# uthree/ALiVE-VC

Hardware: AMD Instinct MI355X
Metric: VC frames/sec + RTF @24kHz, 1M-vec library; 1/2/4/8 MI355X (higher is better)
Workload: dtype decoder fp16 GEMMs / fp32 acc; encoders 22-bit fp16 split; kNN exact fp32 top-k via fp6 MFMA candidates (certified); f32 MFMA small convs; f64 phase scan

## Files before the change

### alive-vc_amd/csrc/gemm_planes.hip

```cpp
#include "conv_epilogue.h"
#include "planes_layout.h"

namespace {

constexpr int GM = 128, GN = 128, GK = 32;
constexpr int PLANE_BYTES = GM * GK * 2;

typedef const __attribute__((address_space(1))) void* gptr_t;
typedef __attribute__((address_space(3))) void* lptr_t;

template <int N>
__device__ __forceinline__ void wait_vmcnt() {
    __builtin_amdgcn_s_waitcnt((N & 15) | (7 << 4) | (15 << 8) | ((N >> 4) << 14));
}
__device__ __forceinline__ void wait_lgkmcnt0() { __builtin_amdgcn_s_waitcnt(15 | (7 << 4) | (0 << 8) | (3 << 14)); }

struct GemmWalk {
    int64_t a_ks, b_blk, b_tap;
    int ncb;
    int rg, n_ct;
};
__device__ __forceinline__ void tile_of(int v, int n_mt, const GemmWalk& g, int& mt, int& ct) {
    const int gs = g.rg * g.n_ct;
    const int grp = v / gs, rem = v - grp * gs;
    const int left = n_mt - grp * g.rg;
    const int rows = left < g.rg ? left : g.rg;
    ct = rem / rows;
    mt = grp * g.rg + (rem - ct * rows);
}
struct StepWalk {
    int64_t a = 0, b = 0;
    int blk = 0;
    __device__ __forceinline__ void reset() { a = 0; b = 0; blk = 0; }
    __device__ __forceinline__ void advance(const GemmWalk& g) {
        a += g.a_ks;
        b += g.b_blk;
        if (++blk == g.ncb) { blk = 0; b += g.b_tap - (int64_t)g.ncb * g.b_blk; }
    }
};

template <int NP>
__device__ __forceinline__ unsigned pack_plane2(float a, float b, bool count = true) { return NP == 1 ? pack_f16x2(a, b, count) : pack_bf16x2(a, b); }
template <int NP, bool F16S>
__device__ __forceinline__ unsigned split_step(float& a, float& b, bool count = true) {
    if constexpr (F16S) {
        typedef _Float16 f16x2_t __attribute__((ext_vector_type(2)));
        const unsigned h = pack_f16x2(a, b, count);
        const f16x2_t hv = __builtin_bit_cast(f16x2_t, h);
        a -= (float)hv[0];
        b -= (float)hv[1];
        return h;
    } else {
        const unsigned h = pack_plane2<NP>(a, b, count);
        a -= __uint_as_float(h << 16);
        b -= __uint_as_float(h & 0xffff0000u);
        return h;
    }
}

template <int NP, int ACT, bool F16S = false>
__device__ __forceinline__ void gemm_epilogue(const AliveGemm& p, f32x16 (&acc)[2][2], int m0, int64_t c0, int wr, int wc, int lr,
                                              int lh, int64_t cols, int64_t cols_pad, int co_pad32, unsigned char* stage = nullptr,
                                              unsigned char* stage_small = nullptr) {
    if constexpr (ACT == 3) {
        float bv[2] = {-INFINITY, -INFINITY};
        int bi[2] = {0x7fffffff, 0x7fffffff};
        auto take = [](float v, int vi, float b, int i) { return argmax_takes(v, vi, b, i); };
#pragma unroll
        for (int ti = 0; ti < 2; ++ti) {
            const int rbase = m0 + wr * 64 + ti * 32 + 4 * lh;
#pragma unroll
            for (int r = 0; r < 16; ++r) {
                const int row = rbase + (r & 3) + 8 * (r >> 2);
                const float b = p.bias != nullptr ? p.bias[row < p.Co ? row : p.Co - 1] : 0.0f;
                const float osc = F16S ? p.wscale[0] * p.in_unscale : 1.0f;
#pragma unroll
                for (int tj = 0; tj < 2; ++tj) {
                    const float x = F16S ? fmaf(acc[ti][tj][r], osc, b) : acc[ti][tj][r] + b;
                    if (row < p.Co && take(x, row, bv[tj], bi[tj])) { bv[tj] = x; bi[tj] = row; }
                }
            }
        }
        const int blk = (m0 + wr * 64) >> 6;
#pragma unroll
        for (int tj = 0; tj < 2; ++tj) {
            const float ov = __shfl_xor(bv[tj], 32);
            const int oi = __shfl_xor(bi[tj], 32);
            if (take(ov, oi, bv[tj], bi[tj])) { bv[tj] = ov; bi[tj] = oi; }
            const int64_t col = c0 + wc * 64 + tj * 32 + lr;
            if (lh == 0 && col < cols && m0 + wr * 64 < p.Co) {
                p.arg_val[(size_t)blk * cols + col] = bv[tj];
                p.arg_idx[(size_t)blk * cols + col] = bi[tj];
            }
        }
        return;
    }
    if constexpr (ACT == 4) {
        unsigned char* st = stage_small != nullptr ? stage_small : stage;
        unsigned short* Po = (unsigned short*)p.Pout;
        const int bins = p.Co >> 1;
        const int bin0 = (m0 + wr * 64) >> 1;
        const int lane = lr + 32 * lh;
#pragma unroll
        for (int tj = 0; tj < 2; ++tj) {
            float q[2][4][2];
#pragma unroll
            for (int ti = 0; ti < 2; ++ti)
#pragma unroll
                for (int g = 0; g < 4; ++g)
#pragma unroll
                    for (int e = 0; e < 2; ++e) {
                        const int bin = bin0 + 16 * ti + 4 * g + 2 * lh + e;
                        const float m = hypotf(acc[ti][tj][4 * g + 2 * e], acc[ti][tj][4 * g + 2 * e + 1]);
                        q[ti][g][e] = bin < bins ? m : 0.0f;
                    }
#pragma unroll
            for (int pl = 0; pl < NP; ++pl) {
#pragma unroll
                for (int ti = 0; ti < 2; ++ti)
#pragma unroll
                    for (int g = 0; g < 4; ++g) {
                        const unsigned h = pack_plane2<NP>(q[ti][g][0], q[ti][g][1]);
                        *(unsigned*)(st + lr * 64 + (((2 * ti + (g >> 1)) ^ ((lr >> 2) & 3)) << 4) + 8 * (g & 1) + 4 * lh) = h;
                        q[ti][g][0] -= __uint_as_float(h << 16);
                        q[ti][g][1] -= __uint_as_float(h & 0xffff0000u);
                    }
#pragma unroll
                for (int it = 0; it < 2; ++it) {
                    const int idx = it * 64 + lane, cl = idx >> 2, chunk = idx & 3;
                    const u32x4 v = *(const u32x4*)(st + cl * 64 + ((chunk ^ ((cl >> 2) & 3)) << 4));
                    const int64_t col = c0 + wc * 64 + tj * 32 + cl;
                    const int b = bin0 + chunk * 8;
                    if (col < cols_pad && b < co_pad32) *(u32x4*)(Po + planes_at(pl, col, b, cols_pad, co_pad32)) = col < cols ? v : u32x4{0u, 0u, 0u, 0u};
                }
            }
        }
        return;
    }
    const bool second = p.y_split > 0 && m0 >= p.y_split;
    float* const Yout = second ? p.Y2 : p.Y;
    const int row_off = second ? p.y_split : 0;
    const int co_out = p.y_split > 0 ? (second ? p.Co - p.y_split : p.y_split) : p.Co;
    unsigned obase[2];
    bool cok[2];
#pragma unroll
    for (int tj = 0; tj < 2; ++tj) {
        const int64_t col = c0 + wc * 64 + tj * 32 + lr;
        cok[tj] = col < cols;
        const int64_t n = cok[tj] ? col / p.T : 0;
        obase[tj] = (unsigned)(n * co_out * p.T + (cok[tj] ? col - n * p.T : 0)) - (unsigned)(row_off * p.T);
    }
    const bool full_rows = m0 + GM <= p.Co;
    const float oscale = F16S ? p.wscale[0] * p.in_unscale : 1.0f;
    const float pscale = F16S ? p.pout_scale : 1.0f;
    const float* __restrict__ bias = p.bias;
    const float* __restrict__ post_add = p.post_add;
    const float* __restrict__ ch_scale = p.ch_scale;
#pragma unroll
    for (int ti = 0; ti < 2; ++ti) {
        const int rbase = m0 + wr * 64 + ti * 32 + 4 * lh;
        float bia[4][4], pad[4][4], scl[4][4];
#pragma unroll
        for (int g = 0; g < 4; ++g)
#pragma unroll
            for (int e = 0; e < 4; ++e) {
                int row = rbase + 8 * g + e;
                row = row < p.Co ? row : p.Co - 1;
                bia[g][e] = bias != nullptr ? bias[row] : 0.0f;
                pad[g][e] = post_add != nullptr ? post_add[row] : 0.0f;
                scl[g][e] = ch_scale != nullptr ? ch_scale[row] : 1.0f;
            }
        float res[2][16];
        if (p.residual != nullptr) {
#pragma unroll
            for (int tj = 0; tj < 2; ++tj)
#pragma unroll
                for (int r = 0; r < 16; ++r) {
                    int row = rbase + (r & 3) + 8 * (r >> 2);
                    row = row < p.Co ? row : p.Co - 1;
                    res[tj][r] = p.residual[obase[tj] + (unsigned)(row * p.T)];
                }
        }
#pragma unroll
        for (int tj = 0; tj < 2; ++tj) {
            float vv[16];
#pragma unroll
            for (int r = 0; r < 16; ++r) {
                float x = F16S ? fmaf(acc[ti][tj][r], oscale, bia[r >> 2][r & 3]) : acc[ti][tj][r] + bia[r >> 2][r & 3];
                if (ACT == 1) x = gelu_fast(x);
                else if (ACT == 2) x = expf(x);
                x = (x + pad[r >> 2][r & 3]) * scl[r >> 2][r & 3];
                if (p.residual != nullptr) x += res[tj][r];
                vv[r] = x;
            }
            if (Yout != nullptr && cok[tj]) {
                if (full_rows) {
#pragma unroll
                    for (int r = 0; r < 16; ++r)
                        Yout[obase[tj] + (unsigned)((rbase + (r & 3) + 8 * (r >> 2)) * p.T)] = vv[r];
                } else {
#pragma unroll
                    for (int r = 0; r < 16; ++r) {
                        const int row = rbase + (r & 3) + 8 * (r >> 2);
                        if (row < p.Co) Yout[obase[tj] + (unsigned)(row * p.T)] = vv[r];
                    }
                }
            }
            if (p.Pout != nullptr && stage != nullptr) {
                const int cl = tj * 32 + lr;
#pragma unroll
                for (int g = 0; g < 4; ++g) {
                    const int rowl = ti * 32 + 8 * g + 4 * lh;
                    float q[4];
#pragma unroll
                    for (int e = 0; e < 4; ++e) q[e] = (full_rows || rbase + 8 * g + e < p.Co) ? vv[4 * g + e] * pscale : 0.0f;
#pragma unroll
                    for (int pl = 0; pl < NP; ++pl) {
                        const unsigned h01 = split_step<NP, F16S>(q[0], q[1], cok[tj]), h23 = split_step<NP, F16S>(q[2], q[3], cok[tj]);
                        *(uint2*)(stage + pl * 8192 + cl * 128 + ((((rowl >> 3)) ^ (cl & 7)) << 4) + 8 * lh) = make_uint2(h01, h23);
                    }
                }
            } else if (p.Pout != nullptr && stage_small != nullptr) {
                unsigned short* Po = (unsigned short*)p.Pout;
                float q[4][4];
#pragma unroll
                for (int g = 0; g < 4; ++g)
#pragma unroll
                    for (int e = 0; e < 4; ++e) q[g][e] = (full_rows || rbase + 8 * g + e < p.Co) ? vv[4 * g + e] * pscale : 0.0f;
                const int lane = lr + 32 * lh;
#pragma unroll
                for (int pl = 0; pl < NP; ++pl) {
#pragma unroll
                    for (int g = 0; g < 4; ++g) {
                        const unsigned h01 = split_step<NP, F16S>(q[g][0], q[g][1], cok[tj]), h23 = split_step<NP, F16S>(q[g][2], q[g][3], cok[tj]);
                        *(uint2*)(stage_small + lr * 64 + ((g ^ ((lr >> 2) & 3)) << 4) + 8 * lh) = make_uint2(h01, h23);
                    }
#pragma unroll
                    for (int it = 0; it < 2; ++it) {
                        const int idx = it * 64 + lane, cl = idx >> 2, chunk = idx & 3;
                        const u32x4 v = *(const u32x4*)(stage_small + cl * 64 + ((chunk ^ ((cl >> 2) & 3)) << 4));
                        const int64_t col = c0 + wc * 64 + tj * 32 + cl;
                        const int row0 = m0 + wr * 64 + ti * 32 + chunk * 8;
                        if (col < cols && row0 < co_pad32) *(u32x4*)(Po + planes_at(pl, col, row0, cols_pad, co_pad32)) = v;
                    }
                }
            }
        }
    }
    if (p.Pout != nullptr && stage != nullptr) {
        unsigned short* Po = (unsigned short*)p.Pout;
        const int lane = lr + 32 * lh;
#pragma unroll
        for (int it = 0; it < 8; ++it) {
            const int cl = (it & 3) * 16 + (lane >> 2), chunk = (it >> 2) * 4 + (lane & 3);
            const int64_t col = c0 + wc * 64 + cl;
            const int row0 = m0 + wr * 64 + chunk * 8;
            if (col >= cols || row0 >= co_pad32) continue;
#pragma unroll
            for (int pl = 0; pl < NP; ++pl) {
                const u32x4 v = *(const u32x4*)(stage + pl * 8192 + cl * 128 + ((chunk ^ (cl & 7)) << 4));
                *(u32x4*)(Po + planes_at(pl, col, row0, cols_pad, co_pad32)) = v;
            }
        }
    }
}

template <int NP, int NS, int MINB, int ACT, bool KB2 = false, bool F16S = false>
__global__ __launch_bounds__(256, MINB) void gemm_planes_kernel(AliveGemm p, int n_mt, int ntiles, int64_t cols,
                                                             int64_t cols_pad, int co_pad, int co_pad32, int kpad,
                                                             GemmWalk gw, long long* stamps) {
#ifdef ALIVE_STAMPS
    const long long ts0 = wall_clock64();
#endif
    extern __shared__ __attribute__((aligned(16))) unsigned char smem[];
    constexpr int SLOT = 2 * NP * PLANE_BYTES;
    constexpr int NI = 4 * NP;
    constexpr int NPROD = KB2 ? 2 : NP * (NP + 1) / 2;
    static_assert(!KB2 || NP == 2, "the 64-deep one-plane form lives in the two-plane kernel's slots");
    static_assert(!F16S || (NP == 2 && !KB2), "fp16 split planes: two planes, 32-deep steps");

    const int tid = threadIdx.x, lane = tid & 63;
    const int w = __builtin_amdgcn_readfirstlane(tid >> 6);
    const int wr = w >> 1, wc = w & 1;
    const int lr = lane & 31, lh = lane >> 5;

    int v;
    {
        const int L = blockIdx.x, xcd = L & 7, j = L >> 3, q = ntiles >> 3, r = ntiles & 7;
        v = (xcd < r ? xcd * (q + 1) : r * (q + 1) + (xcd - r) * q) + j;
    }
    int mt, ct;
    tile_of(v, n_mt, gw, mt, ct);
    const int m0 = mt * GM;
    const int64_t c0 = (int64_t)ct * GN;
    const int nsteps = kpad / (KB2 ? 2 * GK : GK);

    const int prow = lane >> 2;
    const int pchunk = (lane & 3) ^ ((prow >> 2) & 3);
    const unsigned short* src[NI];
    int ldst[NI];
#pragma unroll
    for (int i = 0; i < NI; ++i) {
        const int q = w + 4 * i;
        const int op = q / (8 * NP), pl = (q % (8 * NP)) / 8, g = q % 8;
        const int spl = KB2 ? 0 : pl;
        const int r = g * 16 + prow;
        if (op == 0) {
            int row = m0 + r;
            row = row < co_pad ? row : co_pad - 1;
            src[i] = (const unsigned short*)p.W + planes_at(spl, row, 0, co_pad, kpad) + pchunk * 8;
        } else if (p.b_row == 0) {
            int64_t col = c0 + r;
            col = col < cols_pad ? col : cols_pad - 1;
            src[i] = (const unsigned short*)p.P + planes_at(spl, col, 0, cols_pad, kpad) + pchunk * 8;
        } else {
            int64_t col = c0 + r;
            col = col < cols ? col : cols - 1;
            const int64_t nn = col / p.T;
            src[i] = (const unsigned short*)p.P + (size_t)spl * p.b_plane + (size_t)nn * p.b_win + (size_t)(col - nn * p.T) * p.b_row + pchunk * 8;
        }
        ldst[i] = (op * NP + pl) * PLANE_BYTES + g * 1024;
    }
    StepWalk walk, walk1;
    if constexpr (KB2) walk1.advance(gw);
    auto issue = [&](int step, int i) {
        const StepWalk& wk = (KB2 && ((i >> 1) & 1)) ? walk1 : walk;
        __builtin_amdgcn_global_load_lds((gptr_t)(src[i] + (i < 2 * NP ? wk.a : wk.b)), (lptr_t)(smem + (step % NS) * SLOT + ldst[i]), 16, 0, 0);
    };
    auto next_step = [&]() {
        walk.advance(gw);
        if constexpr (KB2) { walk.advance(gw); walk1.advance(gw); walk1.advance(gw); }
    };

    f32x16 acc[2][2];
#pragma unroll
    for (int i = 0; i < 2; ++i)
#pragma unroll
        for (int r = 0; r < 16; ++r) { acc[i][0][r] = 0.0f; acc[i][1][r] = 0.0f; }

#pragma unroll
    for (int s = 0; s < NS; ++s)
        if (s < nsteps) {
#pragma unroll
            for (int i = 0; i < NI; ++i) issue(s, i);
            next_step();
        }

    const int sw = (lr >> 2) & 3;
    const int a_off = (wr * 64 + lr) * 64 + ((lh ^ sw) << 4);
    const int b_off = NP * PLANE_BYTES + (wc * 64 + lr) * 64 + ((lh ^ sw) << 4);

    bf16x8 fa[2][2][NP], fb[2][2][NP];
    auto load_frags = [&](int step, int ks, bf16x8 (&a)[2][NP], bf16x8 (&b)[2][NP]) {
        const unsigned char* S = smem + (step % NS) * SLOT;
#pragma unroll
        for (int t = 0; t < 2; ++t)
#pragma unroll
            for (int pl = 0; pl < NP; ++pl) {
                a[t][pl] = *(const bf16x8*)(S + ((a_off + t * 2048) ^ (ks << 5)) + pl * PLANE_BYTES);
                b[t][pl] = *(const bf16x8*)(S + ((b_off + t * 2048) ^ (ks << 5)) + pl * PLANE_BYTES);
            }
    };
    auto mma = [&](bf16x8 (&a)[2][NP], bf16x8 (&b)[2][NP], auto&& hook) {
        int n = 0;
        if constexpr (KB2) {
#pragma unroll
            for (int kb = 0; kb < 2; ++kb) {
#pragma unroll
                for (int ti = 0; ti < 2; ++ti)
#pragma unroll
                    for (int tj = 0; tj < 2; ++tj) acc[ti][tj] = mfma_f16(a[ti][kb], b[tj][kb], acc[ti][tj]);
                hook(n++);
            }
            return;
        }
#pragma unroll
        for (int sum = NP - 1; sum >= 0; --sum)
#pragma unroll
            for (int i = 0; i <= sum; ++i) {
#pragma unroll
                for (int ti = 0; ti < 2; ++ti)
#pragma unroll
                    for (int tj = 0; tj < 2; ++tj)
                        acc[ti][tj] = (NP == 1 || F16S) ? mfma_f16(a[ti][i], b[tj][sum - i], acc[ti][tj])
                                                        : __builtin_amdgcn_mfma_f32_32x32x16_bf16(a[ti][i], b[tj][sum - i], acc[ti][tj], 0, 0, 0);
                hook(n++);
            }
    };

#ifdef ALIVE_STAMPS
    const long long ts1 = wall_clock64();
#endif
    if (nsteps >= NS) wait_vmcnt<(NS - 1) * NI>(); else wait_vmcnt<0>();
    __builtin_amdgcn_s_barrier();
    load_frags(0, 0, fa[0], fb[0]);
#ifdef ALIVE_STAMPS
    const long long ts2 = wall_clock64();
    long long cy_vm = 0, cy_bar = 0;
    const long long cy_l0 = __builtin_readcyclecounter();
#endif

    for (int s = 0; s < nsteps; ++s) {
        mma(fa[0], fb[0], [&](int n) {
            if (n == 0) load_frags(s, 1, fa[1], fb[1]);
        });
        __builtin_amdgcn_sched_barrier(0);
        wait_lgkmcnt0();
#ifdef ALIVE_STAMPS
        const long long cy0 = __builtin_readcyclecounter();
#endif
        if (s + NS - 1 < nsteps) wait_vmcnt<(NS - 2) * NI>(); else wait_vmcnt<0>();
#ifdef ALIVE_STAMPS
        const long long cy1 = __builtin_readcyclecounter();
#endif
        __builtin_amdgcn_s_barrier();
#ifdef ALIVE_STAMPS
        const long long cy2 = __builtin_readcyclecounter();
        cy_vm += cy1 - cy0; cy_bar += cy2 - cy1;
#endif
        if (s + 1 < nsteps) load_frags(s + 1, 0, fa[0], fb[0]);
        __builtin_amdgcn_sched_barrier(0);
        const bool refill = s + NS < nsteps;
        mma(fa[1], fb[1], [&](int n) {
#pragma unroll
            for (int i = 0; i < NI; ++i)
                if (i * NPROD / NI == n && refill) issue(s + NS, i);
        });
        next_step();
        __builtin_amdgcn_sched_barrier(0);
    }
    wait_vmcnt<0>();
#ifdef ALIVE_STAMPS
    const long long ts3 = wall_clock64();
    const long long cy_l1 = __builtin_readcyclecounter();
#endif

    unsigned char* stage = nullptr;
    if constexpr (ACT != 3) {
        if (p.Pout != nullptr) {
            __syncthreads();
            stage = smem + w * (NP * 8192);
        }
    }
    gemm_epilogue<KB2 ? 1 : NP, ACT, F16S>(p, acc, m0, c0, wr, wc, lr, lh, cols, cols_pad, co_pad32, stage);
#ifdef ALIVE_STAMPS
    if (stamps != nullptr && tid == 0) {
        long long* o = stamps + (size_t)blockIdx.x * 8;
        o[0] = ts0; o[1] = ts1; o[2] = ts2; o[3] = ts3; o[4] = wall_clock64();
        o[5] = cy_l1 - cy_l0;
        o[6] = cy_vm; o[7] = cy_bar;
    }
#endif
}

template <int NP, int NS, int ACT>
__global__ __launch_bounds__(512, 1) void gemm_planes_lw_kernel(AliveGemm p, int n_mt, int ntiles, int64_t cols, int64_t cols_pad,
                                                                int co_pad, int co_pad32, int kpad, GemmWalk gw) {
    extern __shared__ __attribute__((aligned(16))) unsigned char smem[];
    constexpr int SLOT = 2 * NP * PLANE_BYTES;
    constexpr int NI = 4 * NP;
    [[maybe_unused]] constexpr int NPROD = NP * (NP + 1) / 2;

    const int tid = threadIdx.x, lane = tid & 63;
    const int w8 = __builtin_amdgcn_readfirstlane(tid >> 6);
    const int nsteps = kpad / GK;

    int v, v_end;
    const int v_stride = gridDim.x >> 3;
    {
        const int xcd = blockIdx.x & 7, j = blockIdx.x >> 3, q = ntiles >> 3, r = ntiles & 7;
        const int beg = xcd < r ? xcd * (q + 1) : r * (q + 1) + (xcd - r) * q;
        v_end = beg + q + (xcd < r ? 1 : 0);
        v = beg + j;
    }
    if (v >= v_end) return;

    if (w8 >= 4) {
        const int w = w8 - 4;
        const int prow = lane >> 2;
        const int pchunk = (lane & 3) ^ ((prow >> 2) & 3);
        int ldst[NI];
        unsigned off[2][NI];
#pragma unroll
        for (int i = 0; i < NI; ++i) {
            const int q = w + 4 * i;
            ldst[i] = ((i >= 2 * NP ? NP : 0) + (q % (8 * NP)) / 8) * PLANE_BYTES + (q % 8) * 1024;
        }
        auto tile_offsets = [&](int tv, unsigned (&o)[NI]) {
            int mt, ct;
            tile_of(tv, n_mt, gw, mt, ct);
            const int64_t c0 = (int64_t)ct * GN;
#pragma unroll
            for (int i = 0; i < NI; ++i) {
                const int q = w + 4 * i;
                const int pl = (q % (8 * NP)) / 8, r = (q % 8) * 16 + prow;
                if (i < 2 * NP) {
                    int row = mt * GM + r;
                    row = row < co_pad ? row : co_pad - 1;
                    o[i] = (unsigned)((planes_at(pl, row, 0, co_pad, kpad) + pchunk * 8) * 2);
                } else if (p.b_row == 0) {
                    int64_t col = c0 + r;
                    col = col < cols_pad ? col : cols_pad - 1;
                    o[i] = (unsigned)((planes_at(pl, col, 0, cols_pad, kpad) + pchunk * 8) * 2);
                } else {
                    int64_t col = c0 + r;
                    col = col < cols ? col : cols - 1;
                    const int64_t nn = col / p.T;
                    o[i] = (unsigned)(((size_t)pl * p.b_plane + (size_t)nn * p.b_win + (size_t)(col - nn * p.T) * p.b_row + pchunk * 8) * 2);
                }
            }
        };
        StepWalk walk;
        auto issue = [&](int which, int slot, int i) {
            const unsigned char* base = i >= 2 * NP ? (const unsigned char*)p.P : (const unsigned char*)p.W;
            __builtin_amdgcn_global_load_lds((gptr_t)(base + off[which][i] + (unsigned)((i >= 2 * NP ? walk.b : walk.a) * 2)),
                                             (lptr_t)(smem + slot * SLOT + ldst[i]), 16, 0, 0);
        };
        int cur = 0, qb = 0;
        tile_offsets(v, off[0]);
#pragma unroll
        for (int s = 0; s < NS; ++s) {
#pragma unroll
            for (int i = 0; i < NI; ++i) issue(0, s, i);
            walk.advance(gw);
        }
        wait_vmcnt<(NS - 1) * NI>();
        __builtin_amdgcn_s_barrier();
        while (true) {
            const int vn = v + v_stride;
            const bool has_next = vn < v_end;
            if (has_next) tile_offsets(vn, off[cur ^ 1]);
            for (int s = 0; s < nsteps; ++s) {
                const int slot = (qb + s) % NS;
                if (s + NS - 1 < nsteps || has_next) wait_vmcnt<(NS - 2) * NI>(); else wait_vmcnt<0>();
                __builtin_amdgcn_s_barrier();
                const int ts = s + NS;
                const bool in_tile = ts < nsteps;
                if (ts == nsteps) walk.reset();
                if (in_tile || has_next) {
#pragma unroll
                    for (int i = 0; i < NI; ++i) issue(in_tile ? cur : (cur ^ 1), slot, i);
                }
                walk.advance(gw);
            }
            if (!has_next) break;
            v = vn;
            cur ^= 1;
            qb = (qb + nsteps) % NS;
        }
        return;
    }

    const int w = w8;
    const int wr = w >> 1, wc = w & 1;
    const int lr = lane & 31, lh = lane >> 5;
    const int sw = (lr >> 2) & 3;
    const int a_off = (wr * 64 + lr) * 64 + ((lh ^ sw) << 4);
    const int b_off = NP * PLANE_BYTES + (wc * 64 + lr) * 64 + ((lh ^ sw) << 4);
    bf16x8 fa[2][2][NP], fb[2][2][NP];
    auto load_frags = [&](int slot, int ks, bf16x8 (&a)[2][NP], bf16x8 (&b)[2][NP]) {
        const unsigned char* S = smem + slot * SLOT;
#pragma unroll
        for (int t = 0; t < 2; ++t)
#pragma unroll
            for (int pl = 0; pl < NP; ++pl) {
                a[t][pl] = *(const bf16x8*)(S + ((a_off + t * 2048) ^ (ks << 5)) + pl * PLANE_BYTES);
                b[t][pl] = *(const bf16x8*)(S + ((b_off + t * 2048) ^ (ks << 5)) + pl * PLANE_BYTES);
            }
    };
    f32x16 acc[2][2];
    auto mma = [&](bf16x8 (&a)[2][NP], bf16x8 (&b)[2][NP], auto&& hook) {
        int n = 0;
#pragma unroll
        for (int sum = NP - 1; sum >= 0; --sum)
#pragma unroll
            for (int i = 0; i <= sum; ++i) {
#pragma unroll
                for (int ti = 0; ti < 2; ++ti)
#pragma unroll
                    for (int tj = 0; tj < 2; ++tj)
                        acc[ti][tj] = NP == 1 ? mfma_f16(a[ti][i], b[tj][sum - i], acc[ti][tj])
                                              : __builtin_amdgcn_mfma_f32_32x32x16_bf16(a[ti][i], b[tj][sum - i], acc[ti][tj], 0, 0, 0);
                hook(n++);
            }
    };

    int qb = 0;
    __builtin_amdgcn_s_barrier();
    while (true) {
        const int vn = v + v_stride;
        const bool has_next = vn < v_end;
#pragma unroll
        for (int i = 0; i < 2; ++i)
#pragma unroll
            for (int r = 0; r < 16; ++r) { acc[i][0][r] = 0.0f; acc[i][1][r] = 0.0f; }
        load_frags(qb, 0, fa[0], fb[0]);
        for (int s = 0; s < nsteps; ++s) {
            const int slot = (qb + s) % NS;
            const int slot1 = slot + 1 == NS ? 0 : slot + 1;
            mma(fa[0], fb[0], [&](int n) {
                if (n == 0) load_frags(slot, 1, fa[1], fb[1]);
            });
            __builtin_amdgcn_sched_barrier(0);
            wait_lgkmcnt0();
            __builtin_amdgcn_s_barrier();
            if (s + 1 < nsteps) load_frags(slot1, 0, fa[0], fb[0]);
            __builtin_amdgcn_sched_barrier(0);
            mma(fa[1], fb[1], [&](int) {});
            __builtin_amdgcn_sched_barrier(0);
        }
        {
            int mt, ct;
            tile_of(v, n_mt, gw, mt, ct);
            gemm_epilogue<NP, ACT>(p, acc, mt * GM, (int64_t)ct * GN, wr, wc, lr, lh, cols, cols_pad, co_pad32, nullptr,
                                   p.Pout != nullptr ? smem + NS * SLOT + w * 2048 : nullptr);
        }
        if (!has_next) break;
        v = vn;
        qb = (qb + nsteps) % NS;
    }
}

template <int NP>
__global__ __launch_bounds__(256) void to_planes_kernel(const float* __restrict__ X, int C, int T, int64_t cols, int64_t cols_pad,
                                                        int c_pad, unsigned short* __restrict__ P) {
    __shared__ float tile[64][65];
    const int lane = threadIdx.x & 63, wv = threadIdx.x >> 6;
    const int64_t col0 = (int64_t)blockIdx.x * 64;
    const int ch0 = blockIdx.y * 64;
    {
        const int64_t col = col0 + lane;
        const bool ok = col < cols;
        const int64_t n = ok ? col / T : 0;
        const int t = ok ? (int)(col - n * T) : 0;
        const float* xc = X + (size_t)n * C * T + t;
        for (int r = wv; r < 64; r += 4) {
            const int c = ch0 + r;
            tile[r][lane] = (ok && c < C) ? xc[(size_t)c * T] : 0.0f;
        }
    }
    __syncthreads();
#pragma unroll
    for (int it = 0; it < 2; ++it) {
        const int item = it * 256 + threadIdx.x;
        const int ck = it * 4 + (item & 3), cl = (item >> 2) & 63;
        const int64_t col = col0 + cl;
        const int c = ch0 + ck * 8;
        if (col >= cols_pad || c >= c_pad) continue;
        float vv[8];
#pragma unroll
        for (int e = 0; e < 8; ++e) vv[e] = tile[ck * 8 + e][cl];
#pragma unroll
        for (int pl = 0; pl < NP; ++pl) {
            u32x4 o;
#pragma unroll
            for (int e = 0; e < 4; ++e) {
                const unsigned h = pack_plane2<NP>(vv[2 * e], vv[2 * e + 1]);
                o[e] = h;
                vv[2 * e] -= __uint_as_float(h << 16);
                vv[2 * e + 1] -= __uint_as_float(h & 0xffff0000u);
            }
            *(u32x4*)(P + planes_at(pl, col, c, cols_pad, c_pad)) = o;
        }
    }
}

long long* g_stamps = nullptr;
inline int64_t pad_cols(int64_t cols) { return (cols + GN - 1) / GN * GN; }
inline int pad32(int c) { return (c + 31) & ~31; }
inline GemmWalk make_walk(const AliveGemm& d) {
    GemmWalk g;
    g.a_ks = (int64_t)((d.Co + 15) & ~15) * GK;
    if (d.b_row == 0) { g.b_blk = pad_cols((int64_t)d.N * d.T) * GK; g.b_tap = 0; g.ncb = pad32(d.Ci) / GK; }
    else if (d.b_cblk == 0) { g.b_blk = 0; g.b_tap = GK; g.ncb = 1; }
    else { g.b_blk = d.b_blk; g.b_tap = GK; g.ncb = d.b_cblk; }
    static const int rg_env = getenv("ALIVE_GEMM_RG") ? atoi(getenv("ALIVE_GEMM_RG")) : 0;
    const int n_mt = cdiv(d.Co, GM);
    const int64_t tile_bytes = (int64_t)GM * pad32(d.Ci) * d.planes * 2;
    int rg = rg_env > 0 ? rg_env : (int)std::max<int64_t>(1, (int64_t)(2.5 * 1048576) / tile_bytes);
    rg = std::min(rg, n_mt);
    const int n_rg = cdiv(n_mt, rg);
    g.rg = cdiv(n_mt, n_rg);
    g.n_ct = cdiv((int64_t)d.N * d.T, GN);
    return g;
}

template <int NP, int NS, int MINB, int ACT, bool KB2 = false, bool F16S = false>
int launch_gemm_act(const AliveGemm& d, hipStream_t s) {
    constexpr int LDS = NS * 2 * NP * PLANE_BYTES;
    {
        static LdsOptIn optin;
        hipError_t e = optin.ensure({(const void*)gemm_planes_kernel<NP, NS, MINB, ACT, KB2, F16S>}, LDS);
        if (e != hipSuccess) {
            alive_set_error("alive_gemm_planes: hipFuncSetAttribute: %s", hipGetErrorString(e));
            return ALIVE_ERR_LAUNCH;
        }
    }
    const int64_t cols = (int64_t)d.N * d.T;
    const int n_mt = cdiv(d.Co, GM), n_ct = cdiv(cols, GN);
    const int ntiles = n_mt * n_ct;
    gemm_planes_kernel<NP, NS, MINB, ACT, KB2, F16S><<<ntiles, 256, LDS, s>>>(
        d, n_mt, ntiles, cols, pad_cols(cols), (d.Co + 15) & ~15, pad32(ACT == 4 ? d.Co / 2 : d.Co), pad32(d.Ci), make_walk(d),
        g_stamps);
    ALIVE_CHECK_LAUNCH("alive_gemm_planes");
    return ALIVE_OK;
}

template <int NP, int NS, int ACT>
int launch_gemm_lw_act(const AliveGemm& d, hipStream_t s) {
    constexpr int LDS = NS * 2 * NP * PLANE_BYTES + 4 * 2048;
    {
        static LdsOptIn optin;
        hipError_t e = optin.ensure({(const void*)gemm_planes_lw_kernel<NP, NS, ACT>}, LDS);
        if (e != hipSuccess) {
            alive_set_error("alive_gemm_planes: hipFuncSetAttribute: %s", hipGetErrorString(e));
            return ALIVE_ERR_LAUNCH;
        }
    }
    const int64_t cols = (int64_t)d.N * d.T;
    const int n_mt = cdiv(d.Co, GM), n_ct = cdiv(cols, GN);
    gemm_planes_lw_kernel<NP, NS, ACT><<<256, 512, LDS, s>>>(d, n_mt, n_mt * n_ct, cols, pad_cols(cols), (d.Co + 15) & ~15,
                                                            pad32(ACT == 4 ? d.Co / 2 : d.Co), pad32(d.Ci), make_walk(d));
    ALIVE_CHECK_LAUNCH("alive_gemm_planes(persistent)");
    return ALIVE_OK;
}

template <int NP, int NS>
int launch_gemm_lw(const AliveGemm& d, hipStream_t s) {
    if constexpr (NP == 3) { if (d.act == 3) return launch_gemm_lw_act<NP, NS, 3>(d, s); }
    if constexpr (NP == 3) { if (d.act == 4) return launch_gemm_lw_act<NP, NS, 4>(d, s); }
    if (d.act == 1) return launch_gemm_lw_act<NP, NS, 1>(d, s);
    if (d.act == 2) return launch_gemm_lw_act<NP, NS, 2>(d, s);
    return launch_gemm_lw_act<NP, NS, 0>(d, s);
}

template <int NP, int NS, int MINB>
int launch_gemm(const AliveGemm& d, hipStream_t s) {
    if constexpr (NP == 3) { if (d.act == 3) return launch_gemm_act<NP, NS, MINB, 3>(d, s); }
    if constexpr (NP == 3) { if (d.act == 4) return launch_gemm_act<NP, NS, MINB, 4>(d, s); }
    if (d.act == 1) return launch_gemm_act<NP, NS, MINB, 1>(d, s);
    if (d.act == 2) return launch_gemm_act<NP, NS, MINB, 2>(d, s);
    return launch_gemm_act<NP, NS, MINB, 0>(d, s);
}

}

namespace {
__global__ __launch_bounds__(256) void argmax_merge_kernel(const float* __restrict__ val, const int* __restrict__ idx, int nblk,
                                                           int64_t cols, float* __restrict__ out) {
    const int64_t col = (int64_t)blockIdx.x * 256 + threadIdx.x;
    if (col >= cols) return;
    float b = val[col];
    int i = idx[col];
    for (int k = 1; k < nblk; ++k) {
        const float v = val[(size_t)k * cols + col];
        const int vi = idx[(size_t)k * cols + col];
        if (argmax_takes(v, vi, b, i)) { b = v; i = vi; }
    }
    out[col] = (float)i;
}
}

extern "C" int alive_argmax_merge(const float* arg_val, const int32_t* arg_idx, int nblk, int64_t cols, float* out, void* stream) {
    ALIVE_CHECK_ARG(arg_val && arg_idx && out && nblk > 0 && cols > 0, "alive_argmax_merge: bad args");
    argmax_merge_kernel<<<(unsigned)((cols + 255) / 256), 256, 0, (hipStream_t)stream>>>(arg_val, arg_idx, nblk, cols, out);
    ALIVE_CHECK_LAUNCH("alive_argmax_merge");
    return ALIVE_OK;
}

extern "C" void alive_debug_set_stamps(long long* p) { g_stamps = p; }

extern "C" size_t alive_planes_bytes(int64_t cols, int C, int planes) {
    return (size_t)planes * (size_t)pad_cols(cols) * pad32(C) * 2;
}

extern "C" int alive_to_planes(const float* X, int N, int C, int T, int planes, void* P, void* stream) {
    ALIVE_CHECK_ARG(X && P && N > 0 && C > 0 && T > 0, "alive_to_planes: bad args");
    ALIVE_CHECK_ARG(planes >= 1 && planes <= 3, "alive_to_planes: planes must be 1 (one fp16 plane), 2 or 3 (split bf16), got %d", planes);
    ALIVE_CHECK_ARG((((uintptr_t)P) & 15) == 0, "alive_to_planes: P must be 16-byte aligned");
    const int64_t cols = (int64_t)N * T, cp = pad_cols(cols);
    const int c_pad = pad32(C);
    dim3 g((unsigned)(cp / 64), cdiv(c_pad, 64));
    if (planes == 1) to_planes_kernel<1><<<g, 256, 0, (hipStream_t)stream>>>(X, C, T, cols, cp, c_pad, (unsigned short*)P);
    else if (planes == 2) to_planes_kernel<2><<<g, 256, 0, (hipStream_t)stream>>>(X, C, T, cols, cp, c_pad, (unsigned short*)P);
    else to_planes_kernel<3><<<g, 256, 0, (hipStream_t)stream>>>(X, C, T, cols, cp, c_pad, (unsigned short*)P);
    ALIVE_CHECK_LAUNCH("alive_to_planes");
    return ALIVE_OK;
}

extern "C" int alive_gemm_planes(const AliveGemm* d, void* stream) {
    ALIVE_CHECK_ARG(d && d->W && d->P, "alive_gemm_planes: null pointer");
    if (d->act == 3) {
        ALIVE_CHECK_ARG((d->planes == 3 || (d->planes == 2 && d->f16s)) && d->arg_val && d->arg_idx && !d->Y && !d->Pout && !d->residual &&
                        !d->post_add && !d->ch_scale,
                        "alive_gemm_planes: act 3 (argmax) takes 3 planes (or fp16 split planes), arg_val / arg_idx and no other output or epilogue term");
    } else if (d->act == 4) {
        ALIVE_CHECK_ARG(d->planes == 3 && d->Pout && !d->Y && !d->bias && !d->residual && !d->post_add && !d->ch_scale && !d->y_split && (d->Co & 1) == 0,
                        "alive_gemm_planes: act 4 (magnitude of row pairs) takes 3 planes, an even Co, Pout and no other output or epilogue term");
    } else {
        ALIVE_CHECK_ARG(d->Y || d->Pout, "alive_gemm_planes: no output");
    }
    ALIVE_CHECK_ARG(d->y_split == 0 || (d->y_split % GM == 0 && d->y_split < d->Co && d->Y && d->Y2 && !d->residual && !d->Pout && d->act != 3),
                    "alive_gemm_planes: y_split must be a multiple of %d below Co, with Y and Y2 and neither residual nor Pout", GM);
    ALIVE_CHECK_ARG(d->N > 0 && d->T > 0 && d->Ci > 0 && d->Co > 0, "alive_gemm_planes: bad shape");
    ALIVE_CHECK_ARG(d->planes >= 1 && d->planes <= 3, "alive_gemm_planes: planes must be 1, 2 or 3, got %d", d->planes);
    ALIVE_CHECK_ARG(d->planes != 1 || (d->act != 3 && d->act != 4), "alive_gemm_planes: one plane (plain fp16) has no argmax / magnitude epilogue");
    ALIVE_CHECK_ARG(d->b_row == 0 || ((d->b_row | d->b_win | d->b_plane) & 7) == 0, "alive_gemm_planes: custom row placement must be in multiples of 8 elements");
    ALIVE_CHECK_ARG(d->b_row == 0 || (d->Ci & 31) == 0, "alive_gemm_planes: custom row placement needs Ci %% 32 == 0");
    ALIVE_CHECK_ARG(d->b_cblk >= 0 && (d->b_cblk == 0 || (d->b_row != 0 && (d->Ci / 32) % d->b_cblk == 0 && (d->b_blk & 7) == 0)),
                    "alive_gemm_planes: b_cblk %d (k-blocks per tap) must divide Ci / 32 = %d, with b_row and b_blk set", d->b_cblk, d->Ci / 32);
    ALIVE_CHECK_ARG(d->act >= 0 && d->act <= 4, "alive_gemm_planes: activation %d", d->act);
    ALIVE_CHECK_ARG(((((uintptr_t)d->W) | ((uintptr_t)d->P) | ((uintptr_t)d->Pout)) & 15) == 0,
                    "alive_gemm_planes: W / P / Pout must be 16-byte aligned");
    ALIVE_CHECK_ARG(!(d->Y || d->residual) || (int64_t)d->N * d->Co * d->T < (1ll << 30),
                    "alive_gemm_planes: fp32 tensor of %lld elements exceeds the 32-bit offsets", (long long)d->N * d->Co * d->T);
    static const int variant = getenv("ALIVE_GEMM_VARIANT") ? atoi(getenv("ALIVE_GEMM_VARIANT")) : 0;
    const int64_t ntiles = (int64_t)cdiv(d->Co, GM) * cdiv((int64_t)d->N * d->T, GN);
    const int nsteps = pad32(d->Ci) / GK;
    const bool can_persist = ntiles >= 512 && variant != 1 &&
                             (d->b_row == 0 ? (int64_t)d->planes * pad_cols((int64_t)d->N * d->T) * pad32(d->Ci)
                                            : (int64_t)d->planes * d->b_plane) * 2 < (1ll << 32);
    if (d->planes == 1) {
        if ((pad32(d->Ci) & 63) == 0 && pad32(d->Ci) >= 128) {
            if (d->act == 1) return launch_gemm_act<2, 2, 2, 1, true>(*d, (hipStream_t)stream);
            if (d->act == 2) return launch_gemm_act<2, 2, 2, 2, true>(*d, (hipStream_t)stream);
            return launch_gemm_act<2, 2, 2, 0, true>(*d, (hipStream_t)stream);
        }
        return launch_gemm<1, 4, 2>(*d, (hipStream_t)stream);
    }
    ALIVE_CHECK_ARG(!d->f16s || (d->planes == 2 && d->wscale != nullptr && d->in_unscale > 0.0f && d->act >= 0 && d->act <= 3 &&
                                 (d->Pout == nullptr || d->pout_scale > 0.0f) && d->y_split == 0),
                    "alive_gemm_planes: f16s (fp16 split planes) takes planes = 2, wscale, in_unscale > 0, act 0 - 3 and pout_scale > 0 with Pout");
    if (d->planes == 2 && d->f16s) {
        if (d->act == 3) return launch_gemm_act<2, 2, 2, 3, false, true>(*d, (hipStream_t)stream);
        if (d->act == 1) return launch_gemm_act<2, 2, 2, 1, false, true>(*d, (hipStream_t)stream);
        if (d->act == 2) return launch_gemm_act<2, 2, 2, 2, false, true>(*d, (hipStream_t)stream);
        return launch_gemm_act<2, 2, 2, 0, false, true>(*d, (hipStream_t)stream);
    }
    if (d->planes == 2) {
        return launch_gemm<2, 2, 2>(*d, (hipStream_t)stream);
    }
    if (can_persist && nsteps >= 3) return launch_gemm_lw<3, 3>(*d, (hipStream_t)stream);
    return launch_gemm<3, 3, 1>(*d, (hipStream_t)stream);
}

ALIVE_F16_SAT_GETTER(alive_f16_sat_gemm)
```

### alive-vc_amd/csrc/networks.hip

```cpp
#include <string.h>

#include <string>
#include <vector>

#include "common.h"
#include "planes_layout.h"

int alive_magnitude(const float* ri, int N, int B, int T, float* out, hipStream_t s);

namespace {

constexpr int BINS = 641, NFFT = 1280, HOP = 320;
constexpr int DFT_ROWS = 1296;
constexpr int CE_C = 512, CE_H = 1536, CE_OUT = 768;
constexpr int PE_C = 256, PE_H = 512, PE_OUT = 4096;
constexpr int DEC_C = 512, DEC_H = 1536, NH = 64, SEG = 320;
constexpr float SR = 16000.0f;
constexpr float NORM_EPS = 1e-4f;
constexpr int F_CH[4] = {256, 64, 16, 8};
constexpr int F_UP[4] = {10, 8, 2, 2};
constexpr int FILM_ROWS = 6 * 2 * (256 + 64 + 16 + 8);
constexpr int F_MODE[4] = {0, 1, 2, 2};
constexpr bool F_SPLIT[4] = {true, true, false, false};

inline int pad16(int x) { return (x + 15) & ~15; }

struct Names {
    std::vector<std::string> v;
    int add(const std::string& s) { v.push_back(s); return (int)v.size() - 1; }
};

void convnext_names(Names& n, const std::string& p, bool adaptive) {
    n.add(p + ".dw_w"); n.add(p + ".dw_b");
    if (!adaptive) { n.add(p + ".norm_gain"); n.add(p + ".norm_offset"); }
    n.add(p + ".pw1.W"); n.add(p + ".pw1.b"); n.add(p + ".pw2.W"); n.add(p + ".pw2.b"); n.add(p + ".scale");
    if (!adaptive) { n.add(p + ".pw1.ws"); n.add(p + ".pw2.ws"); }
}

const Names& names_of(int model) {
    static Names ce, pe, dec;
    static const bool init = [&]() {
        ce.add("input.W"); ce.add("input.b");
        for (int i = 0; i < 4; ++i) convnext_names(ce, "mid" + std::to_string(i), false);
        ce.add("output.W"); ce.add("output.b");
        pe.add("input.W"); pe.add("input.b");
        for (int i = 0; i < 4; ++i) convnext_names(pe, "mid" + std::to_string(i), false);
        pe.add("last_norm.gain"); pe.add("last_norm.offset"); pe.add("output.W"); pe.add("output.b"); pe.add("output.ws");
        dec.add("fe.input.W"); dec.add("fe.input.b");
        dec.add("fe.f0c1.W"); dec.add("fe.f0c1.b"); dec.add("fe.f0c2.W"); dec.add("fe.f0c2.b");
        dec.add("fe.normfilm.W"); dec.add("fe.normfilm.b");
        for (int i = 0; i < 4; ++i) convnext_names(dec, "fe.mid" + std::to_string(i), true);
        dec.add("osc.amps.W"); dec.add("osc.amps.b");
        dec.add("flt.film.W"); dec.add("flt.film.b"); dec.add("flt.film.post");
        dec.add("flt.in.W"); dec.add("flt.in.b");
        for (int i = 0; i < 4; ++i) {
            dec.add("flt.down" + std::to_string(i) + ".W"); dec.add("flt.down" + std::to_string(i) + ".b");
            if (i >= 2) dec.add("flt.down" + std::to_string(i) + ".Wp");
        }
        dec.add("flt.mid.W"); dec.add("flt.mid.b");
        for (int i = 0; i < 4; ++i) {
            dec.add("flt.up" + std::to_string(i) + ".W"); dec.add("flt.up" + std::to_string(i) + ".b");
            if (F_MODE[i] == 1) { dec.add("flt.up" + std::to_string(i) + ".Wc"); dec.add("flt.up" + std::to_string(i) + ".bc"); }
        }
        for (int s = 0; s < 4; ++s) {
            std::string b = "flt.blk" + std::to_string(s);
            if (F_MODE[s] == 2) { dec.add(b + ".pack"); continue; }
            if (F_MODE[s] == 1) { dec.add(b + ".packW"); dec.add(b + ".packB"); }
            for (int j = 0; j < 3; ++j)
                for (int c = 1; c <= 2; ++c) {
                    std::string q = b + "." + std::to_string(j) + ".c" + std::to_string(c);
                    dec.add(q + ".W"); dec.add(q + ".b");
                }
        }
        dec.add("flt.out.W"); dec.add("flt.out.b");
        return true;
    }();
    (void)init;
    return model == 0 ? ce : (model == 1 ? pe : dec);
}

struct Table {
    const float* const* w;
    int pos;
    explicit Table(const float* const* p) : w(p), pos(0) {}
    const float* next() { return w[pos++]; }
};

AliveConv conv_desc(const float* W, const float* b, const float* X, int N, int Ci, int Tin, int Co, int KW, int stride,
                    int dil, int pad_left, int pad_mode, int Tout, float* Y) {
    AliveConv d;
    memset(&d, 0, sizeof(d));
    d.W = W; d.bias = b; d.X = X; d.N = N; d.Ci = Ci; d.Tin = Tin; d.Co = Co; d.K_pad = pad16(Ci * KW);
    d.KW = KW; d.stride = stride; d.dil = dil; d.pad_left = pad_left; d.pad_mode = pad_mode; d.Tout = Tout;
    d.up = 1; d.Y = Y;
    return d;
}
AliveConv pw_desc(const float* W, const float* b, const float* X, int N, int Ci, int T, int Co, float* Y) {
    return conv_desc(W, b, X, N, Ci, T, Co, 1, 1, 1, 0, 0, T, Y);
}

AliveConv split(AliveConv d) {
    d.precision = 1;
    d.Ci_pad = (d.Ci + 31) & ~31;
    return d;
}

int g_decoder_precision = 0;
int decoder_precision() {
    if (g_decoder_precision == 0) {
        const char* e = getenv("ALIVE_DECODER_PRECISION");
        g_decoder_precision = (e != nullptr && atoi(e) == 2) ? 2 : 1;
    }
    return g_decoder_precision;
}
int decoder_bf16_mask() {
    return decoder_precision() == 1 ? 23 : 0;
}

bool fb64s_enabled() {
    static const bool on = !(getenv("ALIVE_FB64S") && atoi(getenv("ALIVE_FB64S")) == 0);
    return on;
}
int fine_fusion_level() {
    static const int level = getenv("ALIVE_FINE_FUSE") ? atoi(getenv("ALIVE_FINE_FUSE")) : 2;
    return level;
}
bool fb256_enabled() {
    static const bool on = !(getenv("ALIVE_FB256") && atoi(getenv("ALIVE_FB256")) == 0);
    return on;
}

const float* plain_w(const float* W, int rows_pad16, int K) {
    return (const float*)((const unsigned short*)W + (size_t)2 * rows_pad16 * K);
}
AliveConv plain(AliveConv d) {
    d.precision = 3;
    d.W = plain_w(d.W, (d.Co + 15) & ~15, d.KW * d.Ci_pad);
    return d;
}

AliveConv split3(AliveConv d) {
    d = split(d);
    d.precision = 2;
    return d;
}

#define RUN(expr)                     \
    do {                              \
        int rc_ = (expr);             \
        if (rc_ != ALIVE_OK) return rc_; \
    } while (0)

struct ConvNeXtW {
    const float *dw_w, *dw_b, *gain, *offset, *pw1W, *pw1b, *pw2W, *pw2b, *scale, *ws1, *ws2;
    ConvNeXtW(Table& t, bool adaptive) {
        dw_w = t.next(); dw_b = t.next();
        gain = offset = ws1 = ws2 = nullptr;
        if (!adaptive) { gain = t.next(); offset = t.next(); }
        pw1W = t.next(); pw1b = t.next(); pw2W = t.next(); pw2b = t.next(); scale = t.next();
        if (!adaptive) { ws1 = t.next(); ws2 = t.next(); }
    }
};

constexpr int64_t PLANES_MIN_COLS = 96;
inline bool use_planes(int N, int T) { return (int64_t)N * T >= PLANES_MIN_COLS; }
inline size_t planes_bytes(int N, int T, int C, int planes) { return align_up(alive_planes_bytes((int64_t)N * T, C, planes), 256); }

int pw_gemm(const float* W, const float* b, const void* P, int N, int T, int Ci, int Co, int planes, int act,
            const float* post_add, const float* ch_scale, const float* residual, float* Y, void* Pout, void* s) {
    AliveGemm g;
    memset(&g, 0, sizeof(g));
    g.W = W; g.bias = b; g.P = P; g.N = N; g.T = T; g.Ci = Ci; g.Co = Co; g.planes = planes; g.act = act;
    g.post_add = post_add; g.ch_scale = ch_scale; g.residual = residual; g.Y = Y; g.Pout = Pout;
    return alive_gemm_planes(&g, s);
}

int g_encoder_precision = 0;
int encoder_precision() {
    if (g_encoder_precision == 0) {
        const char* e = getenv("ALIVE_ENCODER_PRECISION");
        g_encoder_precision = (e != nullptr && atoi(e) == 2) ? 2 : 1;
    }
    return g_encoder_precision;
}
constexpr float F16S_ACT_SCALE = 256.0f;

int convnext_layer(const ConvNeXtW& w, float* x, float* ybuf, float* hbuf, void* Pa, void* Ph, int N, int C, int H, int T,
                   const float* cond, int cond_rows, int scale_row, int shift_row, int planes, void* s) {
    if (Pa != nullptr && planes == 3 && w.ws1 != nullptr && encoder_precision() == 1) {
        RUN(alive_dwconv_norm_planes_f16s(x, N, C, T, w.dw_w, w.dw_b, cond ? 1 : 0, w.gain, w.offset, cond, cond_rows, scale_row,
                                          shift_row, NORM_EPS, F16S_ACT_SCALE, Pa, s));
        AliveGemm g;
        memset(&g, 0, sizeof(g));
        g.W = (const float*)((const unsigned short*)w.pw1W + (size_t)3 * ((H + 15) & ~15) * ((C + 31) & ~31));
        g.bias = w.pw1b; g.P = Pa; g.N = N; g.T = T; g.Ci = C; g.Co = H; g.planes = 2; g.act = 1; g.Pout = Ph;
        g.f16s = 1; g.wscale = w.ws1; g.in_unscale = 1.0f / F16S_ACT_SCALE; g.pout_scale = F16S_ACT_SCALE;
        RUN(alive_gemm_planes(&g, s));
        memset(&g, 0, sizeof(g));
        g.W = (const float*)((const unsigned short*)w.pw2W + (size_t)3 * ((C + 15) & ~15) * ((H + 31) & ~31));
        g.bias = w.pw2b; g.P = Ph; g.N = N; g.T = T; g.Ci = H; g.Co = C; g.planes = 2; g.act = 0;
        g.ch_scale = w.scale; g.residual = x; g.Y = x;
        g.f16s = 1; g.wscale = w.ws2; g.in_unscale = 1.0f / F16S_ACT_SCALE;
        return alive_gemm_planes(&g, s);
    }
    if (Pa != nullptr) {
        const int gp = (planes == 2 && (decoder_bf16_mask() & 2)) ? 1 : planes;
        RUN(alive_dwconv_norm_planes(x, N, C, T, w.dw_w, w.dw_b, cond ? 1 : 0, w.gain, w.offset, cond, cond_rows, scale_row,
                                     shift_row, NORM_EPS, gp, Pa, s));
        const float* W1 = gp == 1 ? plain_w(w.pw1W, (H + 15) & ~15, (C + 31) & ~31) : w.pw1W;
        const float* W2 = gp == 1 ? plain_w(w.pw2W, (C + 15) & ~15, (H + 31) & ~31) : w.pw2W;
        RUN(pw_gemm(W1, w.pw1b, Pa, N, T, C, H, gp, 1, nullptr, nullptr, nullptr, nullptr, Ph, s));
        return pw_gemm(W2, w.pw2b, Ph, N, T, H, C, gp, 0, nullptr, w.scale, x, x, nullptr, s);
    }
    RUN(alive_dwconv_norm(x, N, C, T, w.dw_w, w.dw_b, cond ? 1 : 0, w.gain, w.offset, cond, cond_rows, scale_row,
                          shift_row, NORM_EPS, ybuf, s));
    AliveConv d1 = pw_desc(w.pw1W, w.pw1b, ybuf, N, C, T, H, hbuf);
    d1.act = 1;
    d1 = planes == 3 ? split3(d1) : split(d1);
    RUN(alive_conv1d(&d1, s));
    AliveConv d2 = pw_desc(w.pw2W, w.pw2b, hbuf, N, H, T, C, x);
    d2.ch_scale = w.scale;
    d2.residual = x;
    d2 = planes == 3 ? split3(d2) : split(d2);
    RUN(alive_conv1d(&d2, s));
    return ALIVE_OK;
}

int pw_conv(const float* W, const float* b, const float* X, void* Pa, int N, int T, int Ci, int Co, int planes, int act,
            const float* post_add, float* Y, void* s) {
    if (Pa != nullptr) {
        RUN(alive_to_planes(X, N, Ci, T, planes, Pa, s));
        return pw_gemm(W, b, Pa, N, T, Ci, Co, planes, act, post_add, nullptr, nullptr, Y, nullptr, s);
    }
    AliveConv d = pw_desc(W, b, X, N, Ci, T, Co, Y);
    d.act = act;
    d.post_add = post_add;
    d = planes == 3 ? split3(d) : split(d);
    return alive_conv1d(&d, s);
}

__global__ void dft_basis_kernel(float* basis) {
    int i = blockIdx.x * blockDim.x + threadIdx.x;
    if (i >= DFT_ROWS * NFFT) return;
    int row = i / NFFT, j = i % NFFT;
    float v = 0.0f;
    if (row < 2 * BINS) {
        int f = row < BINS ? row : row - BINS;
        int ph = (int)(((long long)f * j) % NFFT);
        double sn, cs;
        sincospi(2.0 * (double)ph / (double)NFFT, &sn, &cs);
        v = row < BINS ? (float)cs : (float)(-sn);
    }
    basis[i] = v;
}

}

extern "C" int alive_weight_count(int model) { return (model >= 0 && model <= 2) ? (int)names_of(model).v.size() : -1; }
extern "C" const char* alive_weight_name(int model, int index) {
    if (model < 0 || model > 2) return nullptr;
    const Names& n = names_of(model);
    return (index >= 0 && index < (int)n.v.size()) ? n.v[index].c_str() : nullptr;
}

int alive_gelu_film_impl(const float* H, int N, int C, int L, const float* film, int film_rows, int Lf, int scale_row,
                         int shift_row, int t0, int f0, int film_ld, float* Z, void* Zp, int planes, void* stream);
namespace {
constexpr size_t BASIS_F32 = (size_t)DFT_ROWS * NFFT;

__global__ void dft_basis_planes_kernel(unsigned short* planes) {
    int i = blockIdx.x * blockDim.x + threadIdx.x;
    if (i >= DFT_ROWS * NFFT) return;
    int row = i / NFFT, j = i % NFFT;
    float v = 0.0f;
    if (row < 2 * BINS) {
        int f = row < BINS ? row : row - BINS;
        int ph = (int)(((long long)f * j) % NFFT);
        double sn, cs;
        sincospi(2.0 * (double)ph / (double)NFFT, &sn, &cs);
        v = row < BINS ? (float)cs : (float)(-sn);
    }
#pragma unroll
    for (int pl = 0; pl < 3; ++pl) {
        const unsigned short h = f32_to_bf16_rn(v);
        planes[planes_at(pl, row, j, DFT_ROWS, NFFT)] = h;
        v -= __uint_as_float((unsigned)h << 16);
    }
}

__global__ void dft_basis_planes_il_kernel(unsigned short* planes) {
    int i = blockIdx.x * blockDim.x + threadIdx.x;
    if (i >= DFT_ROWS * NFFT) return;
    int row = i / NFFT, j = i % NFFT;
    float v = 0.0f;
    if (row < 2 * BINS) {
        int f = row >> 1;
        int ph = (int)(((long long)f * j) % NFFT);
        double sn, cs;
        sincospi(2.0 * (double)ph / (double)NFFT, &sn, &cs);
        v = (row & 1) == 0 ? (float)cs : (float)(-sn);
    }
#pragma unroll
    for (int pl = 0; pl < 3; ++pl) {
        const unsigned short h = f32_to_bf16_rn(v);
        planes[planes_at(pl, row, j, DFT_ROWS, NFFT)] = h;
        v -= __uint_as_float((unsigned)h << 16);
    }
}

__global__ void wav_to_planes_kernel(const float* __restrict__ wav, int L, int Lpad, size_t plane_stride, unsigned short* __restrict__ P) {
    const int i = blockIdx.x * blockDim.x + threadIdx.x;
    if (i >= Lpad) return;
    const int n = blockIdx.y;
    int sidx = i - NFFT / 2;
    sidx = sidx < 0 ? -sidx : sidx;
    sidx = sidx >= L ? 2 * (L - 1) - sidx : sidx;
    float v = wav[(size_t)n * L + sidx];
#pragma unroll
    for (int pl = 0; pl < 3; ++pl) {
        const unsigned short h = f32_to_bf16_rn(v);
        P[(size_t)pl * plane_stride + (size_t)n * Lpad + i] = h;
        v -= __uint_as_float((unsigned)h << 16);
    }
}
}

extern "C" size_t alive_dft_basis_bytes(void) { return BASIS_F32 * sizeof(float) + 2 * 3 * BASIS_F32 * sizeof(unsigned short); }
extern "C" int alive_dft_basis(float* basis, void* stream) {
    ALIVE_CHECK_ARG(basis, "alive_dft_basis: null");
    dft_basis_kernel<<<cdiv((int64_t)DFT_ROWS * NFFT, 256), 256, 0, (hipStream_t)stream>>>(basis);
    dft_basis_planes_kernel<<<cdiv((int64_t)DFT_ROWS * NFFT, 256), 256, 0, (hipStream_t)stream>>>((unsigned short*)(basis + BASIS_F32));
    dft_basis_planes_il_kernel<<<cdiv((int64_t)DFT_ROWS * NFFT, 256), 256, 0, (hipStream_t)stream>>>((unsigned short*)(basis + BASIS_F32) + 3 * BASIS_F32);
    ALIVE_CHECK_LAUNCH("alive_dft_basis");
    return ALIVE_OK;
}
extern "C" size_t alive_spectrogram_workspace_bytes(int N, int L) {
    return align_up((size_t)N * 2 * BINS * (L / HOP) * sizeof(float), 256) + align_up((size_t)3 * N * (L + NFFT) * 2, 256) + 512;
}
extern "C" int alive_spectrogram(const float* basis, const float* wav, int N, int L, float* spec, void* ws, void* stream) {
    ALIVE_CHECK_ARG(basis && wav && spec && ws, "alive_spectrogram: null pointer");
    ALIVE_CHECK_ARG(N > 0 && L > NFFT / 2 && L >= HOP, "alive_spectrogram: needs L > %d samples (reflect pad), got %d", NFFT / 2, L);
    const int T = L / HOP;
    Arena a(ws);
    float* ri = a.take<float>((size_t)N * 2 * BINS * T);
    if (use_planes(N, T) && L % 8 == 0) {
        const int Lpad = L + NFFT;
        unsigned short* wp = a.take<unsigned short>((size_t)3 * N * Lpad);
        wav_to_planes_kernel<<<dim3(cdiv(Lpad, 256), N), 256, 0, (hipStream_t)stream>>>(wav, L, Lpad, (size_t)N * Lpad, wp);
        AliveGemm g;
        memset(&g, 0, sizeof(g));
        g.W = basis + BASIS_F32; g.P = wp; g.N = N; g.T = T; g.Ci = NFFT; g.Co = 2 * BINS; g.planes = 3; g.Y = ri;
        g.b_plane = (int64_t)N * Lpad; g.b_win = Lpad; g.b_row = HOP;
        RUN(alive_gemm_planes(&g, stream));
        return alive_magnitude(ri, N, BINS, T, spec, (hipStream_t)stream);
    }
    AliveConv d = conv_desc(basis, nullptr, wav, N, 1, L, 2 * BINS, NFFT, HOP, 1, NFFT / 2, 2, T, ri);
    RUN(alive_conv1d(&d, stream));
    return alive_magnitude(ri, N, BINS, T, spec, (hipStream_t)stream);
}

namespace {
struct EncBuffers {
    float *x, *y, *h, *lg;
    void *Pa, *Ph;
    size_t bytes;
};
EncBuffers enc_layout(void* ws, int N, int T, int C, int H, int logits) {
    Arena a(ws);
    EncBuffers b;
    const size_t f = (size_t)N * T;
    b.x = a.take<float>(f * C);
    b.y = a.take<float>(f * C);
    b.lg = logits ? a.take<float>(f * logits) : nullptr;
    if (use_planes(N, T)) {
        b.h = nullptr;
        b.Pa = a.take<char>(planes_bytes(N, T, BINS, 3));
        b.Ph = a.take<char>(planes_bytes(N, T, H, 3));
    } else {
        b.h = a.take<float>(f * H);
        b.Pa = b.Ph = nullptr;
    }
    b.bytes = a.used() + 1024;
    return b;
}
}

namespace {
int ce_body(Table& t, EncBuffers& b, int N, int T, float* out, void* stream);
int pe_body(Table& t, EncBuffers& b, int N, int T, float* f0, void* stream, float* logits = nullptr);
}

extern "C" size_t alive_content_encoder_workspace_bytes(int N, int T) { return enc_layout(nullptr, N, T, CE_C, CE_H, 0).bytes; }
extern "C" int alive_content_encoder(const float* const* w, const float* spec, int N, int T, float* out, void* ws, void* stream) {
    ALIVE_CHECK_ARG(w && spec && out && ws && N > 0 && T > 0, "alive_content_encoder: bad args");
    Table t(w);
    EncBuffers b = enc_layout(ws, N, T, CE_C, CE_H, 0);
    const float* inW = t.next(); const float* inb = t.next();
    RUN(pw_conv(inW, inb, spec, b.Pa, N, T, BINS, CE_C, 3, 0, nullptr, b.x, stream));
    return ce_body(t, b, N, T, out, stream);
}
namespace {
int ce_body(Table& t, EncBuffers& b, int N, int T, float* out, void* stream) {
    for (int i = 0; i < 4; ++i) {
        ConvNeXtW cw(t, false);
        RUN(convnext_layer(cw, b.x, b.y, b.h, b.Pa, b.Ph, N, CE_C, CE_H, T, nullptr, 0, 0, 0, 3, stream));
    }
    const float* oW = t.next(); const float* ob = t.next();
    return pw_conv(oW, ob, b.x, b.Pa, N, T, CE_C, CE_OUT, 3, 0, nullptr, out, stream);
}
}

extern "C" size_t alive_f0_estimate_workspace_bytes(int N, int T) { return enc_layout(nullptr, N, T, PE_C, PE_H, PE_OUT).bytes; }
extern "C" int alive_f0_estimate(const float* const* w, const float* spec, int N, int T, float* f0, void* ws, void* stream) {
    ALIVE_CHECK_ARG(w && spec && f0 && ws && N > 0 && T > 0, "alive_f0_estimate: bad args");
    Table t(w);
    EncBuffers b = enc_layout(ws, N, T, PE_C, PE_H, PE_OUT);
    const float* inW = t.next(); const float* inb = t.next();
    RUN(pw_conv(inW, inb, spec, b.Pa, N, T, BINS, PE_C, 3, 0, nullptr, b.x, stream));
    return pe_body(t, b, N, T, f0, stream);
}
extern "C" int alive_f0_logits(const float* const* w, const float* spec, int N, int T, float* logits, void* ws, void* stream) {
    ALIVE_CHECK_ARG(w && spec && logits && ws && N > 0 && T > 0, "alive_f0_logits: bad args");
    Table t(w);
    EncBuffers b = enc_layout(ws, N, T, PE_C, PE_H, PE_OUT);
    const float* inW = t.next(); const float* inb = t.next();
    RUN(pw_conv(inW, inb, spec, b.Pa, N, T, BINS, PE_C, 3, 0, nullptr, b.x, stream));
    return pe_body(t, b, N, T, nullptr, stream, logits);
}
namespace {
int pe_body(Table& t, EncBuffers& b, int N, int T, float* f0, void* stream, float* logits) {
    for (int i = 0; i < 4; ++i) {
        ConvNeXtW cw(t, false);
        RUN(convnext_layer(cw, b.x, b.y, b.h, b.Pa, b.Ph, N, PE_C, PE_H, T, nullptr, 0, 0, 0, 3, stream));
    }
    const float* g = t.next(); const float* of = t.next();
    const float* oW = t.next(); const float* ob = t.next(); const float* ows = t.next();
    if (b.Pa != nullptr && encoder_precision() == 1) {
        RUN(alive_dwconv_norm_planes_f16s(b.x, N, PE_C, T, nullptr, nullptr, 0, g, of, nullptr, 0, 0, 0, NORM_EPS, F16S_ACT_SCALE, b.Pa, stream));
        const int64_t cols = (int64_t)N * T;
        const int nblk = (PE_OUT + 63) / 64;
        AliveGemm gm;
        memset(&gm, 0, sizeof(gm));
        gm.W = (const float*)((const unsigned short*)oW + (size_t)3 * ((PE_OUT + 15) & ~15) * ((PE_C + 31) & ~31));
        gm.bias = ob; gm.P = b.Pa; gm.N = N; gm.T = T; gm.Ci = PE_C; gm.Co = PE_OUT; gm.planes = 2; gm.act = 3;
        gm.f16s = 1; gm.wscale = ows; gm.in_unscale = 1.0f / F16S_ACT_SCALE;
        if (logits != nullptr) {
            gm.act = 0; gm.Y = logits;
            return alive_gemm_planes(&gm, stream);
        }
        gm.arg_val = b.lg;
        gm.arg_idx = (int32_t*)(b.lg + (size_t)nblk * cols);
        RUN(alive_gemm_planes(&gm, stream));
        return alive_argmax_merge(gm.arg_val, gm.arg_idx, nblk, cols, f0, stream);
    }
    if (b.Pa != nullptr) {
        RUN(alive_dwconv_norm_planes(b.x, N, PE_C, T, nullptr, nullptr, 0, g, of, nullptr, 0, 0, 0, NORM_EPS, 3, b.Pa, stream));
        const int nblk = (PE_OUT + 63) / 64;
        const int64_t cols = (int64_t)N * T;
        AliveGemm g;
        memset(&g, 0, sizeof(g));
        g.W = oW; g.bias = ob; g.P = b.Pa; g.N = N; g.T = T; g.Ci = PE_C; g.Co = PE_OUT; g.planes = 3; g.act = 3;
        if (logits != nullptr) {
            g.act = 0; g.Y = logits;
            return alive_gemm_planes(&g, stream);
        }
        g.arg_val = b.lg;
        g.arg_idx = (int32_t*)(b.lg + (size_t)nblk * cols);
        RUN(alive_gemm_planes(&g, stream));
        return alive_argmax_merge(g.arg_val, g.arg_idx, nblk, cols, f0, stream);
    } else {
        RUN(alive_channel_norm(b.x, N, PE_C, T, g, of, NORM_EPS, b.y, stream));
        RUN(pw_conv(oW, ob, b.y, b.Pa, N, T, PE_C, PE_OUT, 3, 0, nullptr, logits != nullptr ? logits : b.lg, stream));
        if (logits != nullptr) return ALIVE_OK;
    }
    return alive_argmax_channels(b.lg, N, PE_OUT, T, f0, stream);
}
}

namespace {
struct FrontBuffers {
    unsigned short* wp;
    char* Ps;
    void *ce_ws, *pe_ws;
    size_t bytes;
};
FrontBuffers front_layout(void* ws, int N, int L) {
    Arena a(ws);
    FrontBuffers b;
    const int T = L / HOP;
    b.wp = a.take<unsigned short>((size_t)3 * N * (L + NFFT));
    b.Ps = a.take<char>(planes_bytes(N, T, BINS, 3));
    b.ce_ws = a.take<char>(enc_layout(nullptr, N, T, CE_C, CE_H, 0).bytes);
    b.pe_ws = a.take<char>(enc_layout(nullptr, N, T, PE_C, PE_H, PE_OUT).bytes);
    b.bytes = a.used() + 1024;
    return b;
}
}
extern "C" size_t alive_front_end_workspace_bytes(int N, int L) { return front_layout(nullptr, N, L).bytes; }
extern "C" int alive_front_end(const float* basis, const float* const* ce_w, const float* const* pe_w, const void* w_in, const float* b_in,
                               const float* wav, int N, int L, float* feat, float* f0, void* ws, void* stream) {
    ALIVE_CHECK_ARG(basis && ce_w && pe_w && w_in && b_in && wav && feat && f0 && ws, "alive_front_end: null pointer");
    ALIVE_CHECK_ARG(N > 0 && L > NFFT / 2 && L >= HOP, "alive_front_end: needs L > %d samples (reflect pad), got %d", NFFT / 2, L);
    const int T = L / HOP;
    ALIVE_CHECK_ARG(use_planes(N, T) && L % 8 == 0, "alive_front_end: batch path only (N * T >= %d frame columns, L %% 8 == 0): use alive_spectrogram + "
                    "alive_f0_estimate + alive_content_encoder", (int)PLANES_MIN_COLS);
    FrontBuffers fb = front_layout(ws, N, L);
    const int Lpad = L + NFFT;
    wav_to_planes_kernel<<<dim3(cdiv(Lpad, 256), N), 256, 0, (hipStream_t)stream>>>(wav, L, Lpad, (size_t)N * Lpad, fb.wp);
    AliveGemm g;
    memset(&g, 0, sizeof(g));
    g.W = (const unsigned short*)(basis + BASIS_F32) + 3 * BASIS_F32; g.P = fb.wp; g.N = N; g.T = T; g.Ci = NFFT; g.Co = 2 * BINS; g.planes = 3;
    g.act = 4; g.Pout = fb.Ps;
    g.b_plane = (int64_t)N * Lpad; g.b_win = Lpad; g.b_row = HOP;
    RUN(alive_gemm_planes(&g, stream));
    EncBuffers ce = enc_layout(fb.ce_ws, N, T, CE_C, CE_H, 0), pe = enc_layout(fb.pe_ws, N, T, PE_C, PE_H, PE_OUT);
    memset(&g, 0, sizeof(g));
    g.W = w_in; g.bias = b_in; g.P = fb.Ps; g.N = N; g.T = T; g.Ci = BINS; g.Co = CE_C + PE_C; g.planes = 3;
    g.Y = ce.x; g.Y2 = pe.x; g.y_split = CE_C;
    RUN(alive_gemm_planes(&g, stream));
    Table tc(ce_w), tp(pe_w);
    tc.next(); tc.next(); tp.next(); tp.next();
    RUN(pe_body(tp, pe, N, T, f0, stream));
    return ce_body(tc, ce, N, T, feat, stream);
}

namespace {
struct DecBuffers {
    float *x, *y, *h, *sinb, *cond, *normfilm, *amps, *src, *film, *d0, *d1, *d2, *d3, *m, *U, *Hh, *Zz, *Z2;
    void *Pa, *Ph;
    void* osc_ws;
    size_t bytes;
};
DecBuffers dec_layout(void* ws, int N, int Lf) {
    Arena a(ws);
    DecBuffers b;
    const size_t f = (size_t)N * Lf, Lw = (size_t)Lf * SEG;
    b.x = a.take<float>(f * DEC_C);
    b.y = a.take<float>(f * DEC_C);
    if (use_planes(N, Lf)) {
        b.h = nullptr;
        b.Pa = a.take<char>(planes_bytes(N, Lf, 768, 2));
        b.Ph = a.take<char>(planes_bytes(N, Lf, DEC_H, 2));
    } else {
        b.h = a.take<float>(f * DEC_H);
        b.Pa = b.Ph = nullptr;
    }
    b.sinb = a.take<float>(f * DEC_C);
    b.cond = a.take<float>(f * DEC_C);
    b.normfilm = a.take<float>(f * 4096);
    b.amps = a.take<float>(f * NH);
    b.src = a.take<float>((size_t)N * Lw);
    b.film = a.take<float>(f * FILM_ROWS);
    b.d0 = a.take<float>((size_t)N * 16 * (Lw / 2));
    b.d1 = a.take<float>((size_t)N * 64 * (Lw / 4));
    b.d2 = a.take<float>((size_t)N * 256 * (Lw / 32));
    b.d3 = a.take<float>(f * 256);
    b.m = a.take<float>(f * 256);
    const size_t big = (size_t)N * 64 * (Lw / 4);
    b.U = a.take<float>(big + 32768);
    b.Hh = a.take<float>(big);
    b.Zz = a.take<float>(big + 32768);
    b.Z2 = a.take<float>(big + 32768);
    b.osc_ws = a.take<char>(alive_oscillator_workspace_bytes(N, NH, Lf));
    b.bytes = a.used() + 1024;
    return b;
}
}

extern "C" size_t alive_decoder_workspace_bytes(int N, int Lf) { return dec_layout(nullptr, N, Lf).bytes; }

namespace {
__global__ void slice_frames_kernel(const float* __restrict__ f0, int Lf, int f_begin, int n_frames, float* __restrict__ out) {
    const int i = blockIdx.x * blockDim.x + threadIdx.x;
    if (i < n_frames) out[(size_t)blockIdx.y * n_frames + i] = f0[(size_t)blockIdx.y * Lf + f_begin + i];
}

int decoder_run(const float* const* w, const float* x_in, const float* f0, const float* f0_win, const float* phi_in, int crop0,
                int phi_col, int N, int Lf, int Lw_frames, int f_begin, float* wave, float* phi_out, DecBuffers& b, void* stream) {
    const bool ranged = Lf != Lw_frames;
    Table t(w);
    const int Lw = Lf * SEG;
    const float* inW = t.next(); const float* inb = t.next();
    RUN(pw_conv(inW, inb, x_in, b.Pa, N, Lf, 768, DEC_C, 2, 0, nullptr, b.x, stream));
    const float* c1W = t.next(); const float* c1b = t.next(); const float* c2W = t.next(); const float* c2b = t.next();
    { AliveConv d = pw_desc(c1W, c1b, f0, N, 1, Lf, DEC_C, b.sinb); d.act = 3; RUN(alive_conv1d(&d, stream)); }
    RUN(pw_conv(c2W, c2b, b.sinb, b.Pa, N, Lf, DEC_C, DEC_C, 2, 0, nullptr, b.cond, stream));
    const float* nfW = t.next(); const float* nfb = t.next();
    if (b.Pa != nullptr && (decoder_bf16_mask() & 4)) {
        RUN(alive_to_planes(b.cond, N, DEC_C, Lf, 1, b.Pa, stream));
        RUN(pw_gemm(plain_w(nfW, 4096, DEC_C), nfb, b.Pa, N, Lf, DEC_C, 4096, 1, 0, nullptr, nullptr, nullptr, b.normfilm, nullptr, stream));
    } else {
        RUN(pw_conv(nfW, nfb, b.cond, b.Pa, N, Lf, DEC_C, 4096, 2, 0, nullptr, b.normfilm, stream));
    }
    for (int i = 0; i < 4; ++i) {
        ConvNeXtW cw(t, true);
        RUN(convnext_layer(cw, b.x, b.y, b.h, b.Pa, b.Ph, N, DEC_C, DEC_H, Lf, b.normfilm, 4096, i * 1024, i * 1024 + 512, 2, stream));
    }
    const float* aW = t.next(); const float* ab = t.next();
    RUN(pw_conv(aW, ab, b.x, b.Pa, N, Lf, DEC_C, NH, 2, 2, nullptr, b.amps, stream));
    RUN(alive_oscillator_range(b.amps, f0_win, phi_in, N, NH, Lw_frames, SEG, SR, crop0, phi_col, f_begin, Lf, b.src, phi_out, b.osc_ws, stream));
    const float* fW = t.next(); const float* fb = t.next(); const float* fpost = t.next();
    if (b.Pa != nullptr) {
        RUN(pw_gemm(fW, fb, b.Pa, N, Lf, DEC_C, FILM_ROWS, 2, 0, fpost, nullptr, nullptr, b.film, nullptr, stream));
    } else {
        AliveConv d = split(pw_desc(fW, fb, b.x, N, DEC_C, Lf, FILM_ROWS, b.film)); d.post_add = fpost; RUN(alive_conv1d(&d, stream));
    }
    const float* siW = t.next(); const float* sib = t.next();
    const int dch[5] = {8, 16, 64, 256, 256};
    const int drate[4] = {2, 2, 8, 10};
    float* dbuf[5] = {nullptr, b.d0, b.d1, b.d2, b.d3};
    {
        const float* W = t.next(); const float* bb = t.next();
        RUN(alive_filter_source_in(b.src, N, Lw, siW, sib, W, bb, b.d0, stream));
    }
    int len = Lw / 2;
    for (int i = 1; i < 4; ++i) {
        const float* W = t.next(); const float* bb = t.next();
        const float* Wp = i >= 2 ? t.next() : nullptr;
        const int r = drate[i];
        if (Wp != nullptr && b.Pa != nullptr) {
            void* Pd = i == 2 ? (void*)b.U : (void*)b.Zz;
            const int cpad = (dch[i] + 31) & ~31;
            AliveGemm g;
            memset(&g, 0, sizeof(g));
            g.W = Wp; g.bias = bb; g.P = Pd; g.N = N; g.T = len / r; g.Ci = r * cpad; g.Co = dch[i + 1];
            g.planes = (decoder_bf16_mask() & 4) ? 1 : 2;
            if (g.planes == 1) g.W = plain_w(Wp, (dch[i + 1] + 15) & ~15, r * cpad);
            g.Y = dbuf[i + 1];
            if (i == 2) g.Pout = b.Zz;
            g.b_plane = (int64_t)(alive_planes_bytes((int64_t)N * len, dch[i], 2) / 4);
            g.b_win = (int64_t)len * 32;
            g.b_row = r * 32;
            g.b_cblk = cpad / 32;
            g.b_blk = g.b_plane / cpad * 32;
            RUN(alive_gemm_planes(&g, stream));
        } else {
            AliveConv d = conv_desc(W, bb, dbuf[i], N, dch[i], len, dch[i + 1], r, r, 1, 0, 0, len / r, dbuf[i + 1]);
            if (i == 1 && b.Pa != nullptr) {
                d.Yp = b.U;
                d.yp_planes = (decoder_bf16_mask() & 4) ? 1 : 2;
            }
            RUN(alive_conv1d(&d, stream));
        }
        len /= r;
    }
    const float* mW = t.next(); const float* mb = t.next();
    {
        AliveConv d = split(conv_desc(mW, mb, b.d3, N, 256, Lf, 256, 5, 1, 1, 4, 1, Lf, b.m));
        if ((decoder_bf16_mask() & 4) && (int64_t)N * Lf > 96) d = plain(d);
        d.skip = b.d3;
        RUN(alive_conv1d(&d, stream));
    }
    const float* upW[4]; const float* upb[4];
    const float* upWc = nullptr; const float* upbc = nullptr;
    for (int i = 0; i < 4; ++i) {
        upW[i] = t.next(); upb[i] = t.next();
        if (F_MODE[i] == 1) { upWc = t.next(); upbc = t.next(); }
    }
    const float* skips[4] = {b.d2, b.d1, b.d0, nullptr};
    const float* cur = b.m;
    int cin = 256, L = Lf, film_off = 0;
    const bool fine = b.Pa != nullptr && fine_fusion_level() >= 1, fine64 = b.Pa != nullptr && fine_fusion_level() >= 2;
    bool folded = false;
    for (int s = 0; s < 4; ++s) {
        const int C = F_CH[s], r = F_UP[s];
        const bool fused256 = F_MODE[s] == 0 && (decoder_bf16_mask() & 1) != 0 && b.Pa != nullptr && fb256_enabled() && L * r >= 128;
        const bool fused64s = F_MODE[s] == 1 && (decoder_bf16_mask() & 16) != 0 && b.Pa != nullptr && fb64s_enabled() && L * r >= 512;
        if (!folded) {
            AliveConv d = conv_desc(fused64s ? upWc : upW[s], fused64s ? upbc : upb[s], cur, N, cin, L, C * r, 1, 1, 1, 0, 0, L,
                                    F_MODE[s] == 0 && !fused256 ? b.Hh : b.U);
            d.up = r;
            if (F_SPLIT[s]) d = split(d);
            RUN(alive_conv1d(&d, stream));
        }
        L *= r;
        const float* blk_in = folded ? cur : b.U;
        float* blk_out = blk_in == b.U ? b.Hh : b.U;
        folded = false;
        if (F_MODE[s] != 0) {
            if (F_MODE[s] == 2) {
                const float* wpack = t.next();
                if (fine && s == 3) {
                    const float* oW = t.next(); const float* ob = t.next();
                    return alive_filter_block_small_wave_range(blk_in, N, L, wpack, b.film, FILM_ROWS, Lw_frames, film_off, f_begin * (L / Lf), f_begin,
                                                               Lf, oW, ob, wave, stream);
                }
                if (fine && s == 2) {
                    RUN(alive_filter_block_small_up_range(blk_in, N, L, wpack, b.film, FILM_ROWS, Lw_frames, film_off, f_begin * (L / Lf), f_begin, Lf,
                                                          skips[s], upW[3], upb[3], blk_out, stream));
                    folded = true;
                } else {
                    RUN(alive_filter_block_small_range(blk_in, N, C, L, wpack, b.film, FILM_ROWS, Lw_frames, film_off, f_begin * (L / Lf), f_begin, Lf,
                                                       skips[s], blk_out, stream));
                }
            } else {
                const float* w16 = t.next(); const float* bias = t.next();
                const void* w6[6]; const float* b6[6];
                for (int q = 0; q < 6; ++q) {
                    w6[q] = plain_w(t.next(), C, 5 * C);
                    b6[q] = t.next();
                }
                if (fused64s && fine64) {
                    RUN(alive_filter_block64s_fp16_up(b.U, N, L, w6, b6, b.film, FILM_ROWS, Lw_frames, film_off, f_begin * (L / Lf), f_begin, Lf, skips[s],
                                                      upW[2], upb[2], b.Hh, b.Zz, (int64_t)N * 64 * (Lw / 4) * 4, stream));
                    folded = true;
                } else if (fused64s)
                    RUN(alive_filter_block64s_fp16(b.U, N, L, w6, b6, b.film, FILM_ROWS, Lw_frames, film_off, f_begin * (L / Lf), f_begin, Lf, skips[s],
                                                   b.Hh, b.Zz, (int64_t)N * 64 * (Lw / 4) * 4, stream));
                else if ((decoder_bf16_mask() & 16) && b.Pa != nullptr)
                    RUN(alive_filter_block64_range_fp16(b.U, N, L, w16, bias, b.film, FILM_ROWS, Lw_frames, film_off, f_begin * (L / Lf), f_begin, Lf,
                                                        skips[s], b.Hh, stream));
                else
                    RUN(alive_filter_block64_range(b.U, N, L, w16, bias, b.film, FILM_ROWS, Lw_frames, film_off, f_begin * (L / Lf), f_begin, Lf,
                                                   skips[s], b.Hh, stream));
            }
            film_off += 6 * 2 * C;
            cur = blk_out;
            cin = C;
            continue;
        }
        if (fused256) {
            const void* w16[6]; const float* bias[6];
            for (int q = 0; q < 6; ++q) {
                w16[q] = plain_w(t.next(), C, 5 * C);
                bias[q] = t.next();
            }
            RUN(alive_filter_block256_fp16(b.U, N, L, w16, bias, b.film, FILM_ROWS, Lw_frames, film_off, f_begin * (L / Lf), f_begin, Lf, skips[s],
                                           b.Hh, b.Zz, (int64_t)N * 64 * (Lw / 4) * 4, stream));
            film_off += 6 * 2 * C;
            cur = b.Hh;
            cin = C;
            continue;
        }
        const bool zplanes = F_SPLIT[s] && (int64_t)N * L > 96 && (L & 3) == 0 && C > 64 && C % 64 == 0 &&
                             (double)(ranged ? Lf : Lw_frames) / (double)L * 128.0 + 3.0 <= 20.0;
        auto set_z = [&](AliveConv& d, float* buf) { if (zplanes) d.Zp = buf; else d.Z = buf; };
        auto set_x = [&](AliveConv& d, const float* buf) { if (zplanes) { d.Xp = buf; d.X = nullptr; } };
        const bool lowp = (decoder_bf16_mask() & 1) != 0 && (int64_t)N * L > 96;
        RUN(alive_gelu_film_impl(b.Hh, N, C, L, b.film, FILM_ROWS, Lw_frames, film_off, film_off + C, ranged ? f_begin * (L / Lf) : 0,
                                 ranged ? f_begin : 0, ranged ? Lf : Lw_frames, zplanes ? nullptr : b.Zz, zplanes ? (void*)b.Zz : nullptr,
                                 lowp ? 1 : 2, stream));
        for (int j = 0; j < 3; ++j) {
            const int dil = 1 << j;
            const float* W1 = t.next(); const float* b1 = t.next(); const float* W2 = t.next(); const float* b2 = t.next();
            const int f1 = film_off + (j * 2) * 2 * C, f2 = film_off + (j * 2 + 1) * 2 * C;
            (void)f1;
            {
                AliveConv d = conv_desc(W1, b1, b.Zz, N, C, L, C, 5, 1, dil, 4 * dil, 1, L, nullptr);
                set_x(d, b.Zz);
                set_z(d, b.Z2); d.film = b.film; d.film_rows = FILM_ROWS; d.Lf = Lw_frames;
            if (ranged) { d.film_t0 = f_begin * (L / Lf); d.film_f0 = f_begin; d.film_ld = Lf; }
                d.film_scale_row = f2; d.film_shift_row = f2 + C;
                if (F_SPLIT[s]) d = split(d);
                if (lowp) d = plain(d);
                RUN(alive_conv1d(&d, stream));
            }
            {
                AliveConv d = conv_desc(W2, b2, b.Z2, N, C, L, C, 5, 1, dil, 4 * dil, 1, L, b.Hh);
                set_x(d, b.Z2);
                d.residual = b.Hh;
                if (j == 2) d.skip = skips[s];
                if (j < 2) {
                    const int fn = film_off + ((j + 1) * 2) * 2 * C;
                    set_z(d, b.Zz); d.film = b.film; d.film_rows = FILM_ROWS; d.Lf = Lw_frames;
            if (ranged) { d.film_t0 = f_begin * (L / Lf); d.film_f0 = f_begin; d.film_ld = Lf; }
                    d.film_scale_row = fn; d.film_shift_row = fn + C;
                }
                if (F_SPLIT[s]) d = split(d);
                if (lowp) d = plain(d);
                RUN(alive_conv1d(&d, stream));
            }
        }
        film_off += 6 * 2 * C;
        cur = b.Hh;
        cin = C;
    }
    const float* oW = t.next(); const float* ob = t.next();
    return alive_filter_source_out(cur, N, Lw, oW, ob, wave, stream);
}
}

extern "C" int alive_decoder_precision(int mode) {
    if (mode == 1 || mode == 2) g_decoder_precision = mode;
    return decoder_precision();
}

int alive_f16_sat_conv_split(int), alive_f16_sat_gemm(int), alive_f16_sat_blocks(int), alive_f16_sat_conv(int), alive_f16_sat_filter_mid(int),
    alive_f16_sat_filter_big(int);
extern "C" int alive_f16_saturations(int reset) {
    const int a = alive_f16_sat_conv_split(reset), b = alive_f16_sat_gemm(reset), c = alive_f16_sat_blocks(reset), d = alive_f16_sat_conv(reset);
    const int e = alive_f16_sat_filter_mid(reset), f = alive_f16_sat_filter_big(reset);
    if (a < 0 || b < 0 || c < 0 || d < 0 || e < 0 || f < 0) return -1;
    const long long t = (long long)a + b + c + d + e + f;
    return (int)(t > 0x7fffffff ? 0x7fffffff : t);
}

int alive_f16_sat_conv_split_clear(void*), alive_f16_sat_gemm_clear(void*), alive_f16_sat_blocks_clear(void*), alive_f16_sat_conv_clear(void*),
    alive_f16_sat_filter_mid_clear(void*), alive_f16_sat_filter_big_clear(void*);
extern "C" int alive_f16_saturations_clear(void* stream) {
    const int r = alive_f16_sat_conv_split_clear(stream) | alive_f16_sat_gemm_clear(stream) | alive_f16_sat_blocks_clear(stream) |
                  alive_f16_sat_conv_clear(stream) | alive_f16_sat_filter_mid_clear(stream) | alive_f16_sat_filter_big_clear(stream);
    if (r != 0) {
        alive_set_error("alive_f16_saturations_clear: the runtime refused the asynchronous clear of a counter");
        return ALIVE_ERR_LAUNCH;
    }
    return ALIVE_OK;
}

extern "C" int alive_encoder_precision(int mode) {
    if (mode == 1 || mode == 2) g_encoder_precision = mode;
    return encoder_precision();
}

extern "C" int alive_decoder_forward(const float* const* w, const float* x_in, const float* f0, const float* phi_in, int crop0,
                                     int phi_col, int N, int Lf, float* wave, float* phi_out, void* ws, void* stream) {
    ALIVE_CHECK_ARG(w && x_in && f0 && wave && ws && N > 0, "alive_decoder_forward: bad args");
    ALIVE_CHECK_ARG(Lf >= 5, "alive_decoder_forward: needs at least 5 frames (reflect pad 4 on the bottleneck), got %d", Lf);
    DecBuffers b = dec_layout(ws, N, Lf);
    return decoder_run(w, x_in, f0, f0, phi_in, crop0, phi_col, N, Lf, Lf, 0, wave, phi_out, b, stream);
}

extern "C" int alive_decoder_forward_range(const float* const* w, const float* x_in, const float* f0, int N, int Lf, int f_begin,
                                           int n_frames, float* wave, void* ws, void* stream) {
    ALIVE_CHECK_ARG(w && x_in && f0 && wave && ws && N > 0, "alive_decoder_forward_range: bad args");
    ALIVE_CHECK_ARG(n_frames >= 5 && f_begin >= 0 && f_begin + n_frames <= Lf, "alive_decoder_forward_range: frames [%d, %d) of %d",
                    f_begin, f_begin + n_frames, Lf);
    DecBuffers b = dec_layout(ws, N, n_frames);
    Arena a((char*)ws + b.bytes);
    b.osc_ws = a.take<char>(alive_oscillator_workspace_bytes(N, NH, Lf));
    float* f0s = a.take<float>((size_t)N * n_frames);
    slice_frames_kernel<<<dim3(cdiv(n_frames, 256), N), 256, 0, (hipStream_t)stream>>>(f0, Lf, f_begin, n_frames, f0s);
    return decoder_run(w, x_in, f0s, f0, nullptr, 0, 0, N, n_frames, Lf, f_begin, wave, nullptr, b, stream);
}
```

### alive-vc_amd/module/_native.py

```python
import ctypes as C
import os

import torch

_HERE = os.path.dirname(os.path.abspath(__file__))
LIB_PATH = os.environ.get("ALIVE_VC_LIB", os.path.join(os.path.dirname(_HERE), "libalive_vc.so"))

_lib = None


class AliveConv(C.Structure):
    _fields_ = [
        ("W", C.c_void_p), ("bias", C.c_void_p), ("X", C.c_void_p),
        ("N", C.c_int), ("Ci", C.c_int), ("Tin", C.c_int), ("Co", C.c_int), ("K_pad", C.c_int),
        ("KW", C.c_int), ("stride", C.c_int), ("dil", C.c_int), ("pad_left", C.c_int), ("pad_mode", C.c_int),
        ("Tout", C.c_int), ("up", C.c_int), ("act", C.c_int),
        ("post_add", C.c_void_p), ("ch_scale", C.c_void_p), ("residual", C.c_void_p), ("skip", C.c_void_p),
        ("Y", C.c_void_p), ("Z", C.c_void_p), ("film", C.c_void_p),
        ("film_rows", C.c_int), ("Lf", C.c_int), ("film_scale_row", C.c_int), ("film_shift_row", C.c_int),
        ("precision", C.c_int), ("Ci_pad", C.c_int),
        ("film_t0", C.c_int), ("film_f0", C.c_int), ("film_ld", C.c_int),
        ("Xp", C.c_void_p), ("Zp", C.c_void_p), ("Yp", C.c_void_p), ("yp_planes", C.c_int),
    ]


class AliveGemm(C.Structure):
    _fields_ = [
        ("W", C.c_void_p), ("bias", C.c_void_p), ("P", C.c_void_p),
        ("N", C.c_int), ("T", C.c_int), ("Ci", C.c_int), ("Co", C.c_int), ("planes", C.c_int), ("act", C.c_int),
        ("post_add", C.c_void_p), ("ch_scale", C.c_void_p), ("residual", C.c_void_p),
        ("Y", C.c_void_p), ("Pout", C.c_void_p),
        ("b_plane", C.c_int64), ("b_win", C.c_int64), ("b_row", C.c_int), ("b_cblk", C.c_int), ("b_blk", C.c_int64),
        ("arg_val", C.c_void_p), ("arg_idx", C.c_void_p),
        ("Y2", C.c_void_p), ("y_split", C.c_int),
        ("f16s", C.c_int), ("wscale", C.c_void_p), ("in_unscale", C.c_float), ("pout_scale", C.c_float),
    ]


_VP, _I, _I64, _F, _D, _SZ = C.c_void_p, C.c_int, C.c_int64, C.c_float, C.c_double, C.c_size_t

PROTOTYPES = {
    "alive_last_error": (C.c_char_p, []),
    "alive_version": (_I, []),
    "alive_library_padded_rows": (_I64, [_I64]),
    "alive_library_pack": (_I, [_VP, _I64, _I, _VP, _VP, _VP, _VP]),
    "alive_knn_workspace_bytes": (_SZ, [_I64, _I64]),
    "alive_knn_workspace_bytes_strict": (_SZ, [_I64, _I64]),
    "alive_knn_workspace_bytes_fast": (_SZ, [_I64, _I64]),
    "alive_knn_search": (_I, [_VP, _I, _I, _VP, _VP, _VP, _I64, _I64, _I, _VP, _VP, _VP, _VP]),
    "alive_library_fp8_bytes": (_SZ, [_I64]),
    "alive_library_rounding_bound": (_I, [_VP, _VP, _VP, _I64, _VP, _VP]),
    "alive_library_pack_lo": (_I, [_VP, _VP, _VP, _I64, _VP, _VP]),
    "alive_knn_search_strict": (_I, [_VP, _I, _I, _VP, _VP, _VP, _VP, _VP, _I64, _I64, _I, _VP, _VP, _VP, _VP, _VP, _VP]),
    "alive_library_pack_fp8": (_I, [_VP, _I64, _VP, _VP]),
    "alive_knn_search_fp8": (_I, [_VP, _I, _I, _VP, _VP, _VP, _VP, _I64, _I64, _I, _VP, _VP, _VP, _VP]),
    "alive_knn_search_stats": (_VP, [_I, _I, _I64, _VP]),
    "alive_debug_knn_stage_view": (_I, [_I64, _I64, _I, _I, _VP, _I]),
    "alive_knn_search_timed": (_I, [_VP, _I, _I, _VP, _VP, _VP, _I64, _I64, _I, _VP, _VP, _VP, _VP, _VP, _VP]),
    "alive_knn_search_fp8_timed": (_I, [_VP, _I, _I, _VP, _VP, _VP, _VP, _I64, _I64, _I, _VP, _VP, _VP, _VP, _VP, _VP]),
    "alive_library_pack_fp6": (_I, [_VP, _I64, _VP, _VP]),
    "alive_knn_sub_coordinates": (_I, []),
    "alive_knn_workspace_bytes_sub": (_SZ, [_I64, _I64]),
    "alive_library_fp6_sub_bytes": (_SZ, [_I64]),
    "alive_library_pack_fp6_sub": (_I, [_VP, _I64, _I64, _I64, _VP, _VP, _VP, _VP]),
    "alive_knn_search_fp6_sub_timed": (_I, [_VP, _VP, _I, _I, _VP, _VP, _VP, _VP, _VP, _VP, _I64, _I64, _I, _VP, _VP, _VP, _VP, _VP, _VP]),
    "alive_knn_rot_coordinates": (_I, []),
    "alive_knn_rot_leading": (_I, []),
    "alive_knn_rot_mixed": (_I, []),
    "alive_library_pack_fp8_rot": (_I, [_VP, _I64, _I64, _I64, _F, _VP, _VP]),
    "alive_knn_search_fp8_rot_timed": (_I, [_VP, _VP, _F, _I, _I, _VP, _VP, _VP, _VP, _I64, _I64, _I, _VP, _VP, _VP, _VP, _VP, _VP]),
    "alive_knn_search_fp6": (_I, [_VP, _I, _I, _VP, _VP, _VP, _VP, _I64, _I64, _I, _VP, _VP, _VP, _VP]),
    "alive_knn_search_fp6_timed": (_I, [_VP, _I, _I, _VP, _VP, _VP, _VP, _I64, _I64, _I, _VP, _VP, _VP, _VP, _VP, _VP]),
    "alive_library_pack_rows": (_I, [_VP, _I64, _I, _VP, _VP, _VP]),
    "alive_knn_grouped_workspace_bytes": (_SZ, [_I, _I, _I]),
    "alive_knn_search_grouped": (_I, [_VP, _I, _I, _VP, _VP, _I64, _VP, _VP, _I, _VP, _VP, _VP, _VP]),
    "alive_knn_merge_gather_rows": (_I, [_VP, _VP, _I, _VP, _VP, _VP, _I, _I, _VP, _VP, _VP]),
    "alive_knn_blend_gather_rows": (_I, [_VP, _VP, _I, _VP, _VP, _VP, _VP, _VP, _I, _I, _VP, _VP]),
    "alive_knn_grouped_k_workspace_bytes": (_SZ, [_I, _I, _I]),
    "alive_knn_search_grouped_k": (_I, [_VP, _I, _I, _VP, _VP, _I64, _VP, _VP, _VP, _I, _VP, _VP, _VP, _VP]),
    "alive_knn_merge_gather_rows_k": (_I, [_VP, _VP, _VP, _I, _VP, _VP, _VP, _I, _I, _VP, _VP, _VP]),
    "alive_knn_blend_gather_rows_k": (_I, [_VP, _VP, _VP, _I, _VP, _VP, _VP, _VP, _VP, _I, _I, _VP, _VP]),
    "alive_pool_append": (_I, [_VP, _I64, _I64, _I64, _I, _VP, _VP, _I64, _I64, _VP, _VP]),
    "alive_pool_move_rows": (_I, [_VP, _VP, _I64, _I64, _I64, _I64, _VP]),
    "alive_pool_image_bytes": (_SZ, [_VP, _I, _VP]),
    "alive_pool_pack_images": (_I, [_VP, _VP, _I64, _VP, _VP, _I, _VP, _VP, _VP]),
    "alive_knn_pool_workspace_bytes": (_SZ, [_I, _I, _I, _I, _I64, _I64]),
    "alive_knn_search_pool": (_I, [_VP, _I, _I, _VP, _VP, _VP, _VP, _VP, _I64, _VP, _VP, _I, _I64, _VP, _I, _VP, _VP, _VP, _VP]),
    "alive_knn_pool_k_workspace_bytes": (_SZ, [_I, _I, _I, _I, _I64, _I64]),
    "alive_knn_search_pool_k": (_I, [_VP, _I, _I, _VP, _VP, _VP, _VP, _VP, _I64, _VP, _VP, _I, _I64, _VP, _VP, _I, _VP, _VP, _VP, _VP]),
    "alive_knn_pool_stats": (_VP, [_VP]),
    "alive_dedup_pass": (_I, [_VP, _VP, _I64, _I, _D, _VP, _VP, _VP]),
    "alive_knn_merge_gather": (_I, [_VP, _VP, _I, _I, _D, _VP, _VP, _I, _I, _VP, _VP, _VP]),
    "alive_conv1d": (_I, [C.POINTER(AliveConv), _VP]),
    "alive_conv1d_tiled": (_I, [C.POINTER(AliveConv), _VP]),
    "alive_conv_up_launches": (_I, [_I]),
    "alive_conv_up_min_blocks": (_I, [_I]),
    "alive_decoder_precision": (_I, [_I]),
    "alive_encoder_precision": (_I, [_I]),
    "alive_f16_saturations": (_I, [_I]),
    "alive_f16_saturations_clear": (_I, [_VP]),
    "alive_gelu_film": (_I, [_VP, _I, _I, _I, _VP, _I, _I, _I, _I, _I, _I, _I, _VP, _VP, _VP]),
    "alive_planes_bytes": (_SZ, [_I64, _I, _I]),
    "alive_to_planes": (_I, [_VP, _I, _I, _I, _I, _VP, _VP]),
    "alive_gemm_planes": (_I, [C.POINTER(AliveGemm), _VP]),
    "alive_argmax_merge": (_I, [_VP, _VP, _I, _I64, _VP, _VP]),
    "alive_filter_block_small_weights": (_I, [_I]),
    "alive_filter_block_small": (_I, [_VP, _I, _I, _I, _VP, _VP, _I, _I, _I, _VP, _VP, _VP]),
    "alive_filter_block_small_range": (_I, [_VP, _I, _I, _I, _VP, _VP, _I, _I, _I, _I, _I, _I, _VP, _VP, _VP]),
    "alive_filter_block_small_up_range": (_I, [_VP, _I, _I, _VP, _VP, _I, _I, _I, _I, _I, _I, _VP, _VP, _VP, _VP, _VP]),
    "alive_filter_block_small_wave_range": (_I, [_VP, _I, _I, _VP, _VP, _I, _I, _I, _I, _I, _I, _VP, _VP, _VP, _VP]),
    "alive_filter_block64_weights": (_I64, []),
    "alive_filter_block64": (_I, [_VP, _I, _I, _VP, _VP, _VP, _I, _I, _I, _VP, _VP, _VP]),
    "alive_filter_block64_range": (_I, [_VP, _I, _I, _VP, _VP, _VP, _I, _I, _I, _I, _I, _I, _VP, _VP, _VP]),
    "alive_filter_block64_range_fp16": (_I, [_VP, _I, _I, _VP, _VP, _VP, _I, _I, _I, _I, _I, _I, _VP, _VP, _VP]),
    "alive_filter_block256_workspace_bytes": (_I64, [_I, _I]),
    "alive_filter_block256_fp16": (_I, [_VP, _I, _I, _VP, _VP, _VP, _I, _I, _I, _I, _I, _I, _VP, _VP, _VP, _I64, _VP]),
    "alive_filter_block64s_workspace_bytes": (_I64, [_I, _I]),
    "alive_filter_block64s_fp16": (_I, [_VP, _I, _I, _VP, _VP, _VP, _I, _I, _I, _I, _I, _I, _VP, _VP, _VP, _I64, _VP]),
    "alive_filter_block64s_fp16_up": (_I, [_VP, _I, _I, _VP, _VP, _VP, _I, _I, _I, _I, _I, _I, _VP, _VP, _VP, _VP, _VP, _I64, _VP]),
    "alive_filter_source_in": (_I, [_VP, _I, _I, _VP, _VP, _VP, _VP, _VP, _VP]),
    "alive_filter_source_out": (_I, [_VP, _I, _I, _VP, _VP, _VP, _VP]),
    "alive_dwconv_norm": (_I, [_VP, _I, _I, _I, _VP, _VP, _I, _VP, _VP, _VP, _I, _I, _I, _F, _VP, _VP]),
    "alive_dwconv_norm_planes": (_I, [_VP, _I, _I, _I, _VP, _VP, _I, _VP, _VP, _VP, _I, _I, _I, _F, _I, _VP, _VP]),
    "alive_dwconv_norm_planes_f16s": (_I, [_VP, _I, _I, _I, _VP, _VP, _I, _VP, _VP, _VP, _I, _I, _I, _F, _F, _VP, _VP]),
    "alive_dwconv_norm_planes_ref": (_I, [_VP, _I, _I, _I, _VP, _VP, _I, _VP, _VP, _VP, _I, _I, _I, _F, _I, _VP, _VP, _F]),
    "alive_channel_norm": (_I, [_VP, _I, _I, _I, _VP, _VP, _F, _VP, _VP]),
    "alive_argmax_channels": (_I, [_VP, _I, _I, _I, _VP, _VP]),
    "alive_oscillator_workspace_bytes": (_SZ, [_I, _I, _I]),
    "alive_oscillator": (_I, [_VP, _VP, _VP, _I, _I, _I, _I, _F, _I, _I, _VP, _VP, _VP, _VP]),
    "alive_oscillator_range": (_I, [_VP, _VP, _VP, _I, _I, _I, _I, _F, _I, _I, _I, _I, _VP, _VP, _VP, _VP]),
    "alive_dft_basis_bytes": (_SZ, []),
    "alive_dft_basis": (_I, [_VP, _VP]),
    "alive_spectrogram_workspace_bytes": (_SZ, [_I, _I]),
    "alive_spectrogram": (_I, [_VP, _VP, _I, _I, _VP, _VP, _VP]),
    "alive_resample_taps": (_I, [_I, _I]),
    "alive_resample_length": (_I64, [_I64, _I, _I]),
    "alive_resample_filter": (_I, [_I, _I, _VP, _VP]),
    "alive_resample": (_I, [_VP, _I, _I, _I, _I, _VP, _F, _F, _VP, _I, _VP]),
    "alive_resample_rows": (_I, [_VP, _I, _I, _I, _I, _VP, _VP, _VP, _VP, _I, _VP]),
    "alive_resample_rows_multi": (_I, [_VP, _I, _I, _VP, _VP, _VP, _I, _VP, _I64, _I, _VP, _VP, _VP, _I, _VP, _VP]),
    "alive_pcm16_to_float": (_I, [_VP, _I64, _VP, _VP]),
    "alive_float_to_pcm16": (_I, [_VP, _I64, _VP, _VP]),
    "alive_weight_count": (_I, [_I]),
    "alive_weight_name": (C.c_char_p, [_I, _I]),
    "alive_front_end_workspace_bytes": (_SZ, [_I, _I]),
    "alive_front_end": (_I, [_VP, _VP, _VP, _VP, _VP, _VP, _I, _I, _VP, _VP, _VP, _VP]),
    "alive_content_encoder_workspace_bytes": (_SZ, [_I, _I]),
    "alive_content_encoder": (_I, [_VP, _VP, _I, _I, _VP, _VP, _VP]),
    "alive_f0_estimate_workspace_bytes": (_SZ, [_I, _I]),
    "alive_f0_estimate": (_I, [_VP, _VP, _I, _I, _VP, _VP, _VP]),
    "alive_f0_logits": (_I, [_VP, _VP, _I, _I, _VP, _VP, _VP]),
    "alive_f0_track_workspace_bytes": (_SZ, [_I, _I, _I]),
    "alive_f0_track_rows": (_I, [_VP, _I, _I, _I, _I, _I, _VP, _VP, _VP, _VP, _VP, _VP, _VP, _VP, _VP, _VP]),
    "alive_decoder_workspace_bytes": (_SZ, [_I, _I]),
    "alive_decoder_forward": (_I, [_VP, _VP, _VP, _VP, _I, _I, _I, _I, _VP, _VP, _VP, _VP]),
    "alive_decoder_forward_range": (_I, [_VP, _VP, _VP, _I, _I, _I, _I, _VP, _VP, _VP]),
    "alive_pitch_transform": (_I, [_VP, _I, _I, _I, _F, _F, _F, _VP]),
    "alive_pitch_transform_rows": (_I, [_VP, _I, _I, _I, _VP, _VP, _VP, _VP]),
    "alive_pitch_stats_groups": (_I, [_VP, _I, _I, _I, _I, _VP, _I, _VP, _VP]),
    "alive_pitch_shift_groups": (_I, [_VP, _VP, _I, _I, _VP, _VP, _VP, _VP, _VP]),
    "alive_pitch_follow_rows": (_I, [_VP, _I, _I, _VP, _VP, _VP, _VP, _VP, _D, _D, _VP, _VP, _VP]),
    "alive_pitch_stats2_groups": (_I, [_VP, _I, _I, _I, _I, _VP, _I, _VP, _VP]),
    "alive_pitch_range_groups": (_I, [_VP, _VP, _I, _I, _VP, _VP, _VP, _D, _VP, _VP, _VP, _VP]),
    "alive_pitch_follow2_rows": (_I, [_VP, _I, _I, _VP, _VP, _VP, _VP, _VP, _VP, _VP, _VP, _D, _D, _D, _VP, _VP, _VP, _VP, _VP, _VP]),
    "alive_pitch_transform_rows_centred": (_I, [_VP, _I, _I, _I, _VP, _VP, _VP, _VP, _VP, _VP]),
    "alive_gate_rows": (_I, [_VP, _I, _I, _I, _I, _VP, _VP, _VP, _VP, _VP, _I, _VP, _VP, _VP, _VP, _VP, _VP, _VP, _VP, _VP]),
    "alive_gate_apply_rows": (_I, [_VP, _I, _I, _VP, _VP, _VP, _VP, _VP]),
    "alive_seam_rows": (_I, [_VP, _I, _I, _VP, _VP, _VP, _VP, _VP, _VP, _VP, _I, _VP, _VP, _VP]),
    "alive_limit_rows": (_I, [_VP, _I, _I, _VP, _VP, _VP, _VP, _VP, _VP, _VP, _VP, _I, _VP, _VP]),
    "alive_limit_waves": (_I, [_VP, _VP, _I, _I, _VP, _I, _I, _VP, _VP, _VP]),
    "alive_loudness_workspace_bytes": (_SZ, [_I, _I]),
    "alive_loudness_measure_waves": (_I, [_VP, _I, _I, _VP, _VP, _VP, _VP, _D, _I, _VP, _VP, _VP, _VP, _SZ, _VP]),
    "alive_loudness_apply_waves": (_I, [_VP, _VP, _I, _I, _VP, _VP, _VP, _VP, _D, _VP, _VP]),
    "alive_loudness_rows": (_I, [_VP, _I, _I, _VP, _VP, _VP, _VP, _VP, _VP, _VP, _VP, _VP]),
    "alive_envelope_waves": (_I,[_VP, _VP, _I, _VP, _I, _I, _VP, _VP, _I, _I, _D, _D, _D, _VP, _VP]),
    "alive_ring_push_rows": (_I, [_VP, _I, _I, _VP, _I, _VP, _VP, _VP, _VP, _I, _I, _VP, _VP, _VP, _VP, _VP]),
    "alive_emit_rows": (_I, [_VP, _I, _I, _VP, _VP, _VP, _VP, _I, _VP]),
    "alive_conceal_rows": (_I, [_VP, _I, _I, _VP, _VP, _I, _VP, _VP, _VP, _VP, _VP, _VP, _VP, _VP, _VP, _VP, _VP, _VP, _I, _VP]),
    "alive_codebook_workspace_bytes": (_SZ, [_I64, _I64]),
    "alive_codebook_update": (_I, [_VP, _I64, _I, _VP, _VP, _I64, _VP, _VP, _VP]),
    "alive_codebook_stats": (_I, [_VP, _VP, _VP, _I64, _VP, _VP, _VP]),
    "alive_world_f0_frames": (_I, [_I, _I, _D]),
    "alive_world_f0_taps_count": (_I, [_I, _D, _D]),
    "alive_world_f0_taps": (_I, [_I, _D, _D, _VP]),
    "alive_world_f0_workspace_bytes": (_SZ, [_I, _I, _I, _D, _D, _D]),
    "alive_world_f0": (_I, [_VP, _I, _I, _I, _D, _D, _D, _VP, _VP, _VP, _SZ, _VP]),
    "alive_world_f0_rows": (_I, [_VP, _I, _I, _I, _D, _D, _D, _VP, _VP, _VP, _VP, _SZ, _VP]),
    "alive_linear_resize": (_I, [_VP, _I, _I, _VP, _I, _VP]),
    "alive_world_f0_stages": (_I, [_VP, _I, _I, _I, _D, _D, _D, _VP, _VP, _VP, _SZ, _I, _VP]),
    "alive_world_f0_layout": (_I, [_I, _I, _I, _D, _D, _D, _VP, _I]),
}


def lib():
    global _lib
    if _lib is None:
        if not os.path.exists(LIB_PATH):
            raise RuntimeError(
                f"{LIB_PATH} not found: the HIP extension is required (no CPU fallback). "
                "Build it with `python -c 'import __graft_entry__ as g; g.build()'`.")
        L = C.CDLL(LIB_PATH)
        for name, (res, args) in PROTOTYPES.items():
            fn = getattr(L, name)
            fn.restype = res
            fn.argtypes = args
        _lib = L
    return _lib


def check(rc, what=""):
    if rc != 0:
        msg = lib().alive_last_error().decode()
        raise ValueError(f"{what}: {msg}" if what else msg)


def ptr(t):
    if t is None:
        return None
    if not t.is_cuda:
        raise RuntimeError("libalive_vc operates on HIP device tensors only (got a CPU tensor)")
    if not t.is_contiguous():
        raise RuntimeError("libalive_vc needs contiguous tensors")
    return t.data_ptr()


def stream():
    return torch.cuda.current_stream().cuda_stream


class Workspace:

    def __init__(self):
        self.bufs = {}

    def get(self, nbytes, device):
        key = (str(device), torch.cuda.current_stream(device).cuda_stream)
        buf = self.bufs.get(key)
        if buf is None or buf.numel() < nbytes:
            buf = torch.empty(int(nbytes), dtype=torch.uint8, device=device)
            self.bufs[key] = buf
        return buf


def weight_names(model):
    L = lib()
    return [L.alive_weight_name(model, i).decode() for i in range(L.alive_weight_count(model))]


class WeightTable:

    def __init__(self, model, packed: dict):
        names = weight_names(model)
        missing = [n for n in names if n not in packed]
        if missing:
            raise KeyError(f"packed weights missing {missing[:4]}...")
        self.tensors = [packed[n] for n in names]
        for n, t in zip(names, self.tensors):
            if t.dtype not in (torch.float32, torch.bfloat16) or not t.is_contiguous() or not t.is_cuda:
                raise RuntimeError(f"packed weight {n} must be a contiguous fp32 / bf16 HIP tensor")
        self.array = (C.c_void_p * len(names))(*[t.data_ptr() for t in self.tensors])
        self.names = names

    def tensor(self, name):
        return self.tensors[self.names.index(name)]
```

### include/alive_vc.h

```cpp
#ifndef ALIVE_VC_H
#define ALIVE_VC_H

#include <stddef.h>
#include <stdint.h>

#ifdef __cplusplus
extern "C" {
#endif

#define ALIVE_OK 0
#define ALIVE_ERR_ARG (-1)
#define ALIVE_ERR_LAUNCH (-2)

#define ALIVE_DIM 768
#define ALIVE_KPRIME 16
#define ALIVE_MAX_K 64

const char* alive_last_error(void);
int alive_version(void);

int64_t alive_library_padded_rows(int64_t M);
int alive_library_pack(const float* tokens_DxM, int64_t M, int D,
                       void* lib_bf16, float* rows_f32, float* norms, void* stream);

size_t alive_knn_workspace_bytes(int64_t Tt, int64_t M);
size_t alive_knn_workspace_bytes_strict(int64_t Tt, int64_t M);
size_t alive_knn_workspace_bytes_fast(int64_t Tt, int64_t M);
int alive_knn_search(const float* src, int N, int T,
                     const void* lib_bf16, const float* rows_f32, const float* norms,
                     int64_t M, int64_t idx_base, int k,
                     float* out_val, int32_t* out_idx, void* ws, void* stream);

int alive_library_rounding_bound(const void* lib_bf16, const float* rows_f32, const float* norms, int64_t M,
                                 float* bound, void* stream);
int alive_library_pack_lo(const void* lib_bf16, const float* rows_f32, const float* norms, int64_t M, void* lib_lo, void* stream);
int alive_knn_search_strict(const float* src, int N, int T,
                            const void* lib_bf16, const void* lib_lo, const float* rows_f32, const float* norms, const float* bound,
                            int64_t M, int64_t idx_base, int k,
                            float* out_val, int32_t* out_idx, void* ws, void* stream, void* ev_start, void* ev_stop);

size_t alive_library_fp8_bytes(int64_t M);
int alive_library_pack_fp8(const void* lib_bf16, int64_t M, void* lib_f8, void* stream);
int alive_knn_search_fp8(const float* src, int N, int T,
                         const void* lib_f8, const void* lib_bf16, const float* rows_f32, const float* norms,
                         int64_t M, int64_t idx_base, int k,
                         float* out_val, int32_t* out_idx, void* ws, void* stream);
const int* alive_knn_search_stats(int N, int T, int64_t M, void* ws);
int alive_debug_knn_stage_view(int64_t Tt, int64_t M, int k, int sub, int64_t* out, int n_out);

int alive_knn_search_timed(const float* src, int N, int T,
                           const void* lib_bf16, const float* rows_f32, const float* norms,
                           int64_t M, int64_t idx_base, int k,
                           float* out_val, int32_t* out_idx, void* ws, void* stream, void* ev_start, void* ev_stop);
int alive_knn_search_fp8_timed(const float* src, int N, int T,
                               const void* lib_f8, const void* lib_bf16, const float* rows_f32, const float* norms,
                               int64_t M, int64_t idx_base, int k,
                               float* out_val, int32_t* out_idx, void* ws, void* stream, void* ev_start, void* ev_stop);

int alive_knn_rot_coordinates(void);
int alive_knn_rot_leading(void);
int alive_knn_rot_mixed(void);
int alive_library_pack_fp8_rot(const float* y_rows, int64_t m0, int64_t count, int64_t M, float c0, void* lib_f8, void* stream);
int alive_knn_search_fp8_rot_timed(const float* src, const float* y_rot, float c0, int N, int T,
                                   const void* lib_f8_rot, const void* lib_bf16, const float* rows_f32, const float* norms,
                                   int64_t M, int64_t idx_base, int k,
                                   float* out_val, int32_t* out_idx, void* ws, void* stream, void* ev_start, void* ev_stop);

int alive_library_pack_fp6(const void* lib_bf16, int64_t M, void* lib_f6, void* stream);
int alive_knn_search_fp6(const float* src, int N, int T,
                         const void* lib_f6, const void* lib_bf16, const float* rows_f32, const float* norms,
                         int64_t M, int64_t idx_base, int k,
                         float* out_val, int32_t* out_idx, void* ws, void* stream);
int alive_knn_search_fp6_timed(const float* src, int N, int T,
                               const void* lib_f6, const void* lib_bf16, const float* rows_f32, const float* norms,
                               int64_t M, int64_t idx_base, int k,
                               float* out_val, int32_t* out_idx, void* ws, void* stream, void* ev_start, void* ev_stop);

int alive_knn_sub_coordinates(void);
size_t alive_knn_workspace_bytes_sub(int64_t Tt, int64_t M);
size_t alive_library_fp6_sub_bytes(int64_t M);
int alive_library_pack_fp6_sub(const float* y_rows, int64_t m0, int64_t count, int64_t M, void* lib_sub, float* rho, int* clip,
                               void* stream);
int alive_knn_search_fp6_sub_timed(const float* src, const float* y_sub, int N, int T, const void* lib_sub, const float* rho,
                                   const void* lib_f6, const void* lib_bf16, const float* rows_f32, const float* norms, int64_t M,
                                   int64_t idx_base, int k, float* out_val, int32_t* out_idx, void* ws, void* stream,
                                   void* ev_start, void* ev_stop);

int alive_knn_merge_gather(const float* cand_val, const int32_t* cand_idx, int n_shards, int k,
                           double alpha, const float* rows_f32_full, const float* src,
                           int N, int T, float* out, int32_t* final_idx, void* stream);

int alive_library_pack_rows(const float* tokens, int64_t M, int Dd, float* rows_f32, float* norms, void* stream);
size_t alive_knn_grouped_workspace_bytes(int N, int T, int k);
int alive_knn_search_grouped(const float* src, int N, int T, const float* rows_f32, const float* norms, int64_t P,
                             const int32_t* seg_lo, const int32_t* seg_len, int k, float* out_val, int32_t* out_idx,
                             void* ws, void* stream);
int alive_knn_merge_gather_rows(const float* cand_val, const int32_t* cand_idx, int k, const double* alpha,
                                const float* rows_f32_full, const float* src, int N, int T, float* out,
                                int32_t* final_idx, void* stream);
#define ALIVE_MAX_BLEND 4
int alive_knn_blend_gather_rows(const float* cand_val, const int32_t* cand_idx, int k, const int32_t* first,
                                const double* weight, const double* alpha, const float* rows_f32_full, const float* src,
                                int N, int T, float* out, void* stream);

size_t alive_knn_grouped_k_workspace_bytes(int N, int T, int k_max);
int alive_knn_search_grouped_k(const float* src, int N, int T, const float* rows_f32, const float* norms, int64_t P,
                               const int32_t* seg_lo, const int32_t* seg_len, const int32_t* k_row, int k_max, float* out_val,
                               int32_t* out_idx, void* ws, void* stream);
int alive_knn_merge_gather_rows_k(const float* cand_val, const int32_t* cand_idx, const int32_t* k_row, int k_max,
                                  const double* alpha, const float* rows_f32_full, const float* src, int N, int T, float* out,
                                  int32_t* final_idx, void* stream);
int alive_knn_blend_gather_rows_k(const float* cand_val, const int32_t* cand_idx, const int32_t* k_row, int k_max,
                                  const int32_t* first, const double* weight, const double* alpha, const float* rows_f32_full,
                                  const float* src, int N, int T, float* out, void* stream);

int alive_pool_append(const float* tokens, int64_t row_stride, int64_t col_stride, int64_t M, int Dd, float* rows_f32,
                      float* norms, int64_t capacity, int64_t at, int32_t* report, void* stream);
int alive_pool_move_rows(float* rows_f32, float* norms, int64_t capacity, int64_t src, int64_t dst, int64_t n, void* stream);

#define ALIVE_POOL_STATS 8
size_t alive_pool_image_bytes(const int32_t* seg_len, int V, int64_t* img_off);
int alive_pool_pack_images(const float* rows_f32, const float* norms, int64_t P, const int32_t* seg_lo, const int32_t* seg_len,
                           int V, void* images, float* bounds, void* stream);
size_t alive_knn_pool_workspace_bytes(int N, int T, int k, int V, int64_t P, int64_t max_len);
int alive_knn_search_pool(const float* src, int N, int T, const void* images, const int64_t* img_off, const float* rows_f32,
                          const float* norms, const float* bounds, int64_t P, const int32_t* seg_lo, const int32_t* seg_len,
                          int V, int64_t max_len, const int32_t* voice, int k, float* out_val, int32_t* out_idx, void* ws,
                          void* stream);
size_t alive_knn_pool_k_workspace_bytes(int N, int T, int k_max, int V, int64_t P, int64_t max_len);
int alive_knn_search_pool_k(const float* src, int N, int T, const void* images, const int64_t* img_off, const float* rows_f32,
                            const float* norms, const float* bounds, int64_t P, const int32_t* seg_lo, const int32_t* seg_len,
                            int V, int64_t max_len, const int32_t* voice, const int32_t* k_row, int k_max, float* out_val,
                            int32_t* out_idx, void* ws, void* stream);
const int* alive_knn_pool_stats(void* ws);

int alive_dedup_pass(const float* val, const int32_t* idx, int64_t M, int k, double threshold, int32_t* state,
                     int32_t* undecided, void* stream);

typedef struct AliveConv {
    const float* W;
    const float* bias;
    const float* X;
    int N, Ci, Tin;
    int Co;
    int K_pad;
    int KW, stride, dil;
    int pad_left;
    int pad_mode;
    int Tout;
    int up;
    int act;
    const float* post_add;
    const float* ch_scale;
    const float* residual;
    const float* skip;
    float* Y;
    float* Z;
    const float* film;
    int film_rows, Lf, film_scale_row, film_shift_row;
    int precision, Ci_pad;
    int film_t0, film_f0, film_ld;
    const void* Xp;
    void* Zp;
    void* Yp;
    int yp_planes;
} AliveConv;
int alive_conv1d(const AliveConv* desc, void* stream);
int alive_conv1d_tiled(const AliveConv* desc, void* stream);
int alive_conv_up_launches(int reset);
int alive_conv_up_min_blocks(int blocks);

size_t alive_planes_bytes(int64_t cols, int C, int planes);
int alive_to_planes(const float* X, int N, int C, int T, int planes, void* P, void* stream);
typedef struct AliveGemm {
    const void* W;
    const float* bias;
    const void* P;
    int N, T;
    int Ci, Co;
    int planes;
    int act;
    const float* post_add;
    const float* ch_scale;
    const float* residual;
    float* Y;
    void* Pout;
    int64_t b_plane, b_win;
    int b_row;
    int b_cblk;
    int64_t b_blk;
    float* arg_val;
    int32_t* arg_idx;
    float* Y2;
    int y_split;
    int f16s;
    const float* wscale;
    float in_unscale, pout_scale;
} AliveGemm;
int alive_gemm_planes(const AliveGemm* desc, void* stream);
int alive_argmax_merge(const float* arg_val, const int32_t* arg_idx, int nblk, int64_t cols, float* out, void* stream);

int alive_filter_block_small_weights(int C);
int alive_filter_block_small(const float* U, int N, int C, int L, const float* wpack, const float* film,
                             int film_rows, int Lf, int film_off, const float* skip, float* out, void* stream);
int alive_filter_block_small_range(const float* U, int N, int C, int L, const float* wpack, const float* film,
                                   int film_rows, int Lf, int film_off, int t0, int f0, int film_ld, const float* skip,
                                   float* out, void* stream);
int alive_filter_block_small_up_range(const float* U, int N, int L, const float* wpack, const float* film, int film_rows, int Lf,
                                      int film_off, int t0, int f0, int film_ld, const float* skip, const float* upW, const float* upb,
                                      float* out, void* stream);
int alive_filter_block_small_wave_range(const float* U, int N, int L, const float* wpack, const float* film, int film_rows, int Lf,
                                        int film_off, int t0, int f0, int film_ld, const float* oW, const float* ob, float* wave,
                                        void* stream);

int64_t alive_filter_block64_weights(void);
int alive_filter_block64(const float* U, int N, int L, const void* W16, const float* biases, const float* film,
                         int film_rows, int Lf, int film_off, const float* skip, float* out, void* stream);
int alive_filter_block64_range(const float* U, int N, int L, const void* W16, const float* biases, const float* film,
                               int film_rows, int Lf, int film_off, int t0, int f0, int film_ld, const float* skip,
                               float* out, void* stream);
int alive_filter_block64_range_fp16(const float* U, int N, int L, const void* W16, const float* biases, const float* film,
                               int film_rows, int Lf, int film_off, int t0, int f0, int film_ld, const float* skip,
                               float* out, void* stream);

int64_t alive_filter_block256_workspace_bytes(int N, int L);
int alive_filter_block256_fp16(const float* U, int N, int L, const void* const* w16, const float* const* bias, const float* film,
                               int film_rows, int Lf, int film_off, int t0, int f0, int film_ld, const float* skip, float* out,
                               void* ws, int64_t ws_bytes, void* stream);

int64_t alive_filter_block64s_workspace_bytes(int N, int L);
int alive_filter_block64s_fp16(const float* U, int N, int L, const void* const* w16, const float* const* bias, const float* film,
                               int film_rows, int Lf, int film_off, int t0, int f0, int film_ld, const float* skip, float* out,
                               void* ws, int64_t ws_bytes, void* stream);
int alive_filter_block64s_fp16_up(const float* U, int N, int L, const void* const* w16, const float* const* bias, const float* film,
                                  int film_rows, int Lf, int film_off, int t0, int f0, int film_ld, const float* skip, const float* upW,
                                  const float* upb, float* out, void* ws, int64_t ws_bytes, void* stream);

int alive_filter_source_in(const float* src, int N, int Lw, const float* Win, const float* bin, const float* Wd,
                           const float* bd, float* d0, void* stream);
int alive_filter_source_out(const float* H, int N, int Lw, const float* W, const float* b, float* wave, void* stream);

int alive_dwconv_norm(const float* X, int N, int C, int T, const float* dw_w, const float* dw_b,
                      int affine_mode, const float* gain, const float* offset,
                      const float* cond, int cond_rows, int scale_row, int shift_row,
                      float eps, float* Y, void* stream);
int alive_dwconv_norm_planes(const float* X, int N, int C, int T, const float* dw_w, const float* dw_b,
                             int affine_mode, const float* gain, const float* offset,
                             const float* cond, int cond_rows, int scale_row, int shift_row,
                             float eps, int planes, void* P, void* stream);
int alive_dwconv_norm_planes_f16s(const float* X, int N, int C, int T, const float* dw_w, const float* dw_b,
                                  int affine_mode, const float* gain, const float* offset,
                                  const float* cond, int cond_rows, int scale_row, int shift_row,
                                  float eps, float scale, void* P, void* stream);
int alive_dwconv_norm_planes_ref(const float* X, int N, int C, int T, const float* dw_w, const float* dw_b,
                                 int affine_mode, const float* gain, const float* offset,
                                 const float* cond, int cond_rows, int scale_row, int shift_row,
                                 float eps, int planes, void* P, void* stream, float f16_scale);
int alive_gelu_film(const float* H, int N, int C, int L, const float* film, int film_rows, int Lf, int scale_row,
                    int shift_row, int t0, int f0, int film_ld, float* Z, void* Zp, void* stream);
int alive_channel_norm(const float* X, int N, int C, int T, const float* gain, const float* offset,
                       float eps, float* Y, void* stream);
int alive_argmax_channels(const float* X, int N, int C, int T, float* out, void* stream);

size_t alive_oscillator_workspace_bytes(int N, int H, int Lf);
int alive_oscillator(const float* amps, const float* f0, const float* phi_in, int N, int H, int Lf,
                     int seg, float sample_rate, int crop0, int phi_col,
                     float* wave, float* phi_out, void* ws, void* stream);
int alive_oscillator_range(const float* amps, const float* f0, const float* phi_in, int N, int H, int Lf,
                           int seg, float sample_rate, int crop0, int phi_col, int f_begin, int n_frames,
                           float* wave, float* phi_out, void* ws, void* stream);

size_t alive_dft_basis_bytes(void);
int alive_dft_basis(float* basis, void* stream);
size_t alive_spectrogram_workspace_bytes(int N, int L);
int alive_spectrogram(const float* basis, const float* wav, int N, int L, float* spec, void* ws, void* stream);

int alive_decoder_forward_range(const float* const* w, const float* x, const float* f0, int N, int Lf, int f_begin,
                                int n_frames, float* wave, void* ws, void* stream);

int alive_resample_taps(int orig, int new_rate);
int64_t alive_resample_length(int64_t L, int orig, int new_rate);
int alive_resample_filter(int orig, int new_rate, float* filt, void* stream);
int alive_resample(const float* x, int B, int L, int orig, int new_rate, const float* filt, float pre_scale,
                   float post_scale, float* y, int Lout, void* stream);
int alive_resample_rows(const float* x, int B, int L, int orig, int new_rate, const float* filt, const float* pre_scale,
                        const float* post_scale, float* y, int Lout, void* stream);
int alive_resample_rows_multi(const float* x, int B, int ld_in, const int* len_in, const int* pair, const int* table, int n_pairs,
                              const float* filt, int64_t filt_len, int lds_bytes, const float* pre_scale, const float* post_scale,
                              float* y, int ld_out, const int* len_out, void* stream);
int alive_pcm16_to_float(const int16_t* in, int64_t n, float* out, void* stream);
int alive_float_to_pcm16(const float* in, int64_t n, int16_t* out, void* stream);

int alive_weight_count(int model);
const char* alive_weight_name(int model, int index);

size_t alive_front_end_workspace_bytes(int N, int L);
int alive_front_end(const float* basis, const float* const* ce_weights, const float* const* pe_weights, const void* w_in,
                    const float* b_in, const float* wav, int N, int L, float* feat, float* f0, void* ws, void* stream);
size_t alive_content_encoder_workspace_bytes(int N, int T);
int alive_content_encoder(const float* const* w, const float* spec, int N, int T,
                          float* out, void* ws, void* stream);

size_t alive_f0_estimate_workspace_bytes(int N, int T);
int alive_f0_estimate(const float* const* w, const float* spec, int N, int T,
                      float* f0, void* ws, void* stream);

int alive_f0_logits(const float* const* w, const float* spec, int N, int T, float* logits, void* ws, void* stream);

#define ALIVE_F0_TRACK_MAX_STATES 4000
size_t alive_f0_track_workspace_bytes(int N, int T, int S);
int alive_f0_track_rows(const float* logits, int N, int C, int T, int lo, int S, const double* semis, const int32_t* band_lo,
                        const int32_t* band_hi, const int32_t* on, const double* weight, const double* jump, float* f0,
                        int32_t* changed, void* ws, void* stream);

int alive_decoder_precision(int mode);
int alive_encoder_precision(int mode);
int alive_f16_saturations(int reset);
int alive_f16_saturations_clear(void* stream);

size_t alive_decoder_workspace_bytes(int N, int Lf);
int alive_decoder_forward(const float* const* w, const float* x, const float* f0,
                          const float* phi_in, int crop0, int phi_col, int N, int Lf,
                          float* wave, float* phi_out, void* ws, void* stream);

int alive_pitch_transform(float* f0, int N, int T, int mode, float f0_rate, float pitch_shift,
                          float intonation, void* stream);
int alive_pitch_transform_rows(float* f0, int N, int T, int mode, const float* f0_rate, const float* pitch_shift,
                               const float* intonation, void* stream);

int alive_pitch_stats_groups(const float* f0, int N, int T, int t_lo, int t_hi, const int* first, int G, double* stats, void* stream);
int alive_pitch_shift_groups(const double* stats, const int* first, int G, int N, const float* offset, const int* auto_on,
                             const float* target, float* shift_out, void* stream);
int alive_pitch_follow_rows(const float* f0, int N, int T, const float* f0_rate, const float* offset, const int* auto_on,
                            const float* target, const unsigned char* emit, double decay, double prior, double* state,
                            float* shift_out, void* stream);

int alive_pitch_stats2_groups(const float* f0, int N, int T, int t_lo, int t_hi, const int* first, int G, double* stats3, void* stream);
int alive_pitch_range_groups(const double* stats3, const int* first, int G, int N, const float* inton, const int* range_on,
                             const double* target_sd, double range_max, float* inton_out, float* centre_out, int* centre_on_out,
                             void* stream);
int alive_pitch_follow2_rows(const float* f0, int N, int T, const float* f0_rate, const float* offset, const int* auto_on,
                             const float* target, const float* inton, const int* range_on, const double* target_sd,
                             const unsigned char* emit, double decay, double prior, double range_max, double* state3, float* shift_out,
                             float* inton_out, float* centre_out, int* centre_on_out, void* stream);
int alive_pitch_transform_rows_centred(float* f0, int N, int T, int mode, const float* f0_rate, const float* shift, const float* inton,
                                       const float* centre, const int* centre_on, void* stream);

int alive_gate_rows(const float* x, int N, int ld, int w_lo, int w_hi, const int* gate_on, const double* thr_ms,
                    const int* hold_ticks, const unsigned char* emit, const int* world_on, int S, const int* seg_len, int* state,
                    float* g0, float* g1, int* seg_len_eff, unsigned char* follow, int* world_eff, double* ms_out, void* stream);
int alive_gate_apply_rows(float* y, int N, int ld, const int* span_lo, const int* span_len, const float* g0, const float* g1,
                          void* stream);

int alive_seam_rows(float* y, int N, int ld, const int* span_lo, const int* shift, const int* xlen, const unsigned char* emit,
                    const float* g0, const float* g1, float* tail, int ld_tail, int* stored, double* stats, void* stream);

#define ALIVE_LIMIT_TILE 1024
#define ALIVE_LIMIT_MAX_HIST 3072
int alive_limit_rows(float* y, int N, int ld, const int* span_lo, const int* span_len, const int* shift, const int* look,
                     const int* hold, const float* ceil, const unsigned char* emit, float* hist, int ld_hist, float* gmin, void* stream);
int alive_limit_waves(float* out, const float* y, int N, int ld, const int* len, int look, int hold, const float* ceil, float* gmin,
                      void* stream);

#define ALIVE_LOUDNESS_STATE 16
#define ALIVE_LOUDNESS_PARAMS 6
size_t alive_loudness_workspace_bytes(int N, int max_tiles);
int alive_loudness_measure_waves(const float* y, int N, int ld, const int* len, const int* hop, const double* coef, const double* ap,
                                 double z_abs, int max_tiles, double* zI, int* c1, int* c2, void* workspace, size_t workspace_bytes,
                                 void* stream);
int alive_loudness_apply_waves(float* out, const float* y, int N, int ld, const int* len, const double* zI, const int* c2,
                               const double* z_t, double gmax, double* gain, void* stream);
int alive_loudness_rows(float* y, int N, int ld, const int* span_lo, const int* span_len, const unsigned char* emit,
                        const unsigned char* on, const int* hop, const double* coef, const double* par, double* state, void* stream);

int alive_ring_push_rows(int16_t* ring, int N, int ld, const int16_t* chunks, int ld_chunk, const int* chunk_len, const int* ring_len,
                         const unsigned char* present, float* x, int ld_x, int S, const int* seg_len, int* seg_len_tick,
                         const int* world_on, int* world_tick, void* stream);
int alive_emit_rows(const float* wave, int N, int ld, const int* span_lo, const int* span_len, const unsigned char* take, int16_t* out,
                    int ld_out, void* stream);

#define ALIVE_CONCEAL_MAX_SPAN 4096
#define ALIVE_CONCEAL_QMAX (1 << 30)
int alive_conceal_rows(const int16_t* ring, int N, int ld, const int* ring_len, int16_t* chunks, int ld_chunk, const int* chunk_len,
                       const unsigned char* present, const unsigned char* lost, const unsigned char* on, const int* lag_lo,
                       const int* lag_hi, const int* window, const int* hold, const int* fade, const int* recover, int* state,
                       int16_t* tmpl, int ld_tmpl, void* stream);

#define ALIVE_ENVELOPE_TILE 16
#define ALIVE_ENVELOPE_MAX_RADIUS 4
int alive_envelope_waves(float* out, const float* y, int ld_y, const float* x, int ld_x, int N, const int* len, const float* amount,
                         int hop, int radius, double floor_ms, double g_lo, double g_hi, float* gain_minmax, void* stream);

size_t alive_codebook_workspace_bytes(int64_t M, int64_t C);
int alive_codebook_update(const float* rows, int64_t M, int Dd, const int32_t* order, const int32_t* seg_off, int64_t C,
                          float* centroids, void* ws, void* stream);
int alive_codebook_stats(const int32_t* assign, const int32_t* prev, const float* val, int64_t M, double* objective, int64_t* moved,
                         void* stream);

int alive_world_f0_frames(int L8, int fs, double frame_period);
int alive_world_f0_taps_count(int fs, double f0_floor, double f0_ceil);
int alive_world_f0_taps(int fs, double f0_floor, double f0_ceil, double* host_taps);
size_t alive_world_f0_workspace_bytes(int N, int L8, int fs, double f0_floor, double f0_ceil, double frame_period);
int alive_world_f0(const float* x8, int N, int L8, int fs, double f0_floor, double f0_ceil, double frame_period,
                   const double* taps, float* f0_out, void* ws, size_t ws_bytes, void* stream);
int alive_world_f0_rows(const float* x8, int N, int L8, int fs, double f0_floor, double f0_ceil, double frame_period,
                        const double* taps, const int32_t* row_on, float* f0_out, void* ws, size_t ws_bytes, void* stream);
int alive_linear_resize(const float* x, int rows, int Lin, float* y, int Lout, void* stream);
int alive_world_f0_stages(const float* x8, int N, int L8, int fs, double f0_floor, double f0_ceil, double frame_period,
                          const double* taps, float* f0_out, void* ws, size_t ws_bytes, int stages, void* stream);
int alive_world_f0_layout(int N, int L8, int fs, double f0_floor, double f0_ceil, double frame_period, int64_t* out, int n_out);

#ifdef __cplusplus
}
#endif
#endif
```

Baseline: 1.326 million.

## Keep activations resident as GEMM operand planes across decoder and encoder layers

Adds a pout_fmt option so a GEMM epilogue writes its output straight into the plane format the next GEMM consumes (bf16 to one fp16 plane, fp16 to bf16 planes, f16-split to three bf16 planes), zero-filling padded columns. Adds a fused sin-activation conv that emits planes directly, and rewires the decoder (and apparently the content encoder) to chain GEMMs through planes instead of writing fp32 tensors and re-converting them. This removes intermediate fp32 writes, reads and separate to-planes conversion launches. The old path is kept behind _ref entry points for checking, and the format conversions may change rounding slightly.

```diff
diff --git a/alive-vc_amd/csrc/gemm_planes.hip b/alive-vc_amd/csrc/gemm_planes.hip
--- a/alive-vc_amd/csrc/gemm_planes.hip
+++ b/alive-vc_amd/csrc/gemm_planes.hip
@@ -58,7 +58,7 @@
     }
 }
 
-template <int NP, int ACT, bool F16S = false>
+template <int NP, int ACT, bool F16S = false, int OF = 0>
 __device__ __forceinline__ void gemm_epilogue(const AliveGemm& p, f32x16 (&acc)[2][2], int m0, int64_t c0, int wr, int wc, int lr,
                                               int lh, int64_t cols, int64_t cols_pad, int co_pad32, unsigned char* stage = nullptr,
                                               unsigned char* stage_small = nullptr) {
@@ -152,7 +152,9 @@
     }
     const bool full_rows = m0 + GM <= p.Co;
     const float oscale = F16S ? p.wscale[0] * p.in_unscale : 1.0f;
-    const float pscale = F16S ? p.pout_scale : 1.0f;
+    constexpr int ONP = OF == 0 ? NP : OF;
+    constexpr bool OF16S = F16S && OF == 0;
+    const float pscale = OF16S ? p.pout_scale : 1.0f;
     const float* __restrict__ bias = p.bias;
     const float* __restrict__ post_add = p.post_add;
     const float* __restrict__ ch_scale = p.ch_scale;
@@ -215,8 +217,8 @@
 #pragma unroll
                     for (int e = 0; e < 4; ++e) q[e] = (full_rows || rbase + 8 * g + e < p.Co) ? vv[4 * g + e] * pscale : 0.0f;
 #pragma unroll
-                    for (int pl = 0; pl < NP; ++pl) {
-                        const unsigned h01 = split_step<NP, F16S>(q[0], q[1], cok[tj]), h23 = split_step<NP, F16S>(q[2], q[3], cok[tj]);
+                    for (int pl = 0; pl < ONP; ++pl) {
+                        const unsigned h01 = split_step<ONP, OF16S>(q[0], q[1], cok[tj]), h23 = split_step<ONP, OF16S>(q[2], q[3], cok[tj]);
                         *(uint2*)(stage + pl * 8192 + cl * 128 + ((((rowl >> 3)) ^ (cl & 7)) << 4) + 8 * lh) = make_uint2(h01, h23);
                     }
                 }
@@ -229,10 +231,10 @@
                     for (int e = 0; e < 4; ++e) q[g][e] = (full_rows || rbase + 8 * g + e < p.Co) ? vv[4 * g + e] * pscale : 0.0f;
                 const int lane = lr + 32 * lh;
 #pragma unroll
-                for (int pl = 0; pl < NP; ++pl) {
+                for (int pl = 0; pl < ONP; ++pl) {
 #pragma unroll
                     for (int g = 0; g < 4; ++g) {
-                        const unsigned h01 = split_step<NP, F16S>(q[g][0], q[g][1], cok[tj]), h23 = split_step<NP, F16S>(q[g][2], q[g][3], cok[tj]);
+                        const unsigned h01 = split_step<ONP, OF16S>(q[g][0], q[g][1], cok[tj]), h23 = split_step<ONP, OF16S>(q[g][2], q[g][3], cok[tj]);
                         *(uint2*)(stage_small + lr * 64 + ((g ^ ((lr >> 2) & 3)) << 4) + 8 * lh) = make_uint2(h01, h23);
                     }
 #pragma unroll
@@ -241,7 +243,8 @@
                         const u32x4 v = *(const u32x4*)(stage_small + cl * 64 + ((chunk ^ ((cl >> 2) & 3)) << 4));
                         const int64_t col = c0 + wc * 64 + tj * 32 + cl;
                         const int row0 = m0 + wr * 64 + ti * 32 + chunk * 8;
-                        if (col < cols && row0 < co_pad32) *(u32x4*)(Po + planes_at(pl, col, row0, cols_pad, co_pad32)) = v;
+                        if (col < (OF != 0 ? cols_pad : cols) && row0 < co_pad32)
+                            *(u32x4*)(Po + planes_at(pl, col, row0, cols_pad, co_pad32)) = (OF == 0 || col < cols) ? v : u32x4{0u, 0u, 0u, 0u};
                     }
                 }
             }
@@ -255,20 +258,19 @@
             const int cl = (it & 3) * 16 + (lane >> 2), chunk = (it >> 2) * 4 + (lane & 3);
             const int64_t col = c0 + wc * 64 + cl;
             const int row0 = m0 + wr * 64 + chunk * 8;
-            if (col >= cols || row0 >= co_pad32) continue;
-#pragma unroll
-            for (int pl = 0; pl < NP; ++pl) {
+            if (col >= (OF != 0 ? cols_pad : cols) || row0 >= co_pad32) continue;
+#pragma unroll
+            for (int pl = 0; pl < ONP; ++pl) {
                 const u32x4 v = *(const u32x4*)(stage + pl * 8192 + cl * 128 + ((chunk ^ (cl & 7)) << 4));
-                *(u32x4*)(Po + planes_at(pl, col, row0, cols_pad, co_pad32)) = v;
-            }
-        }
-    }
-}
-
-template <int NP, int NS, int MINB, int ACT, bool KB2 = false, bool F16S = false>
-__global__ __launch_bounds__(256, MINB) void gemm_planes_kernel(AliveGemm p, int n_mt, int ntiles, int64_t cols,
-                                                             int64_t cols_pad, int co_pad, int co_pad32, int kpad,
-                                                             GemmWalk gw, long long* stamps) {
+                *(u32x4*)(Po + planes_at(pl, col, row0, cols_pad, co_pad32)) = (OF == 0 || col < cols) ? v : u32x4{0u, 0u, 0u, 0u};
+            }
+        }
+    }
+}
+
+template <int NP, int NS, int ACT, bool KB2, bool F16S, int OF>
+__device__ __forceinline__ void gemm_planes_tile(const AliveGemm& p, int n_mt, int ntiles, int64_t cols, int64_t cols_pad, int co_pad,
+                                                 int co_pad32, int kpad, const GemmWalk& gw, long long* stamps) {
 #ifdef ALIVE_STAMPS
     const long long ts0 = wall_clock64();
 #endif
@@ -435,14 +437,15 @@
     const long long cy_l1 = __builtin_readcyclecounter();
 #endif
 
-    unsigned char* stage = nullptr;
+    unsigned char *stage = nullptr, *stage_small = nullptr;
     if constexpr (ACT != 3) {
         if (p.Pout != nullptr) {
             __syncthreads();
-            stage = smem + w * (NP * 8192);
-        }
-    }
-    gemm_epilogue<KB2 ? 1 : NP, ACT, F16S>(p, acc, m0, c0, wr, wc, lr, lh, cols, cols_pad, co_pad32, stage);
+            if constexpr (OF <= NP) stage = smem + w * (NP * 8192);
+            else stage_small = smem + w * 2048;
+        }
+    }
+    gemm_epilogue<KB2 ? 1 : NP, ACT, F16S, OF>(p, acc, m0, c0, wr, wc, lr, lh, cols, cols_pad, co_pad32, stage, stage_small);
 #ifdef ALIVE_STAMPS
     if (stamps != nullptr && tid == 0) {
         long long* o = stamps + (size_t)blockIdx.x * 8;
@@ -451,6 +454,19 @@
         o[6] = cy_vm; o[7] = cy_bar;
     }
 #endif
+}
+
+template <int NP, int NS, int MINB, int ACT, bool KB2 = false, bool F16S = false>
+__global__ __launch_bounds__(256, MINB) void gemm_planes_kernel(AliveGemm p, int n_mt, int ntiles, int64_t cols,
+                                                             int64_t cols_pad, int co_pad, int co_pad32, int kpad,
+                                                             GemmWalk gw, long long* stamps) {
+    gemm_planes_tile<NP, NS, ACT, KB2, F16S, 0>(p, n_mt, ntiles, cols, cols_pad, co_pad, co_pad32, kpad, gw, stamps);
+}
+template <int NP, int NS, int MINB, int ACT, bool KB2, bool F16S, int OF>
+__global__ __launch_bounds__(256, MINB) void gemm_planes_fmt_kernel(AliveGemm p, int n_mt, int ntiles, int64_t cols,
+                                                                 int64_t cols_pad, int co_pad, int co_pad32, int kpad,
+                                                                 GemmWalk gw, long long* stamps) {
+    gemm_planes_tile<NP, NS, ACT, KB2, F16S, OF>(p, n_mt, ntiles, cols, cols_pad, co_pad, co_pad32, kpad, gw, stamps);
 }
 
 template <int NP, int NS, int ACT>
@@ -654,12 +670,34 @@
         for (int pl = 0; pl < NP; ++pl) {
             u32x4 o;
 #pragma unroll
-            for (int e = 0; e < 4; ++e) {
-                const unsigned h = pack_plane2<NP>(vv[2 * e], vv[2 * e + 1]);
-                o[e] = h;
-                vv[2 * e] -= __uint_as_float(h << 16);
-                vv[2 * e + 1] -= __uint_as_float(h & 0xffff0000u);
-            }
+            for (int e = 0; e < 4; ++e) o[e] = split_step<NP, false>(vv[2 * e], vv[2 * e + 1]);
+            *(u32x4*)(P + planes_at(pl, col, c, cols_pad, c_pad)) = o;
+        }
+    }
+}
+
+__global__ __launch_bounds__(256) void sin_planes_kernel(const float* __restrict__ W, int w_ld, const float* __restrict__ bias,
+                                                         const float* __restrict__ x, int C, int64_t cols, int64_t cols_pad, int c_pad,
+                                                         unsigned short* __restrict__ P) {
+    const int64_t col0 = (int64_t)blockIdx.x * 64;
+    const int ch0 = blockIdx.y * 64;
+#pragma unroll
+    for (int it = 0; it < 2; ++it) {
+        const int item = it * 256 + threadIdx.x;
+        const int ck = it * 4 + (item & 3), cl = (item >> 2) & 63;
+        const int64_t col = col0 + cl;
+        const int c = ch0 + ck * 8;
+        if (col >= cols_pad || c >= c_pad) continue;
+        const float xv = col < cols ? x[col] : 0.0f;
+        float vv[8];
+#pragma unroll
+        for (int e = 0; e < 8; ++e)
+            vv[e] = (col < cols && c + e < C) ? apply_act(fmaf(W[(size_t)(c + e) * w_ld], xv, bias != nullptr ? bias[c + e] : 0.0f) + 0.0f, 3) : 0.0f;
+#pragma unroll
+        for (int pl = 0; pl < 2; ++pl) {
+            u32x4 o;
+#pragma unroll
+            for (int e = 0; e < 4; ++e) o[e] = split_step<2, false>(vv[2 * e], vv[2 * e + 1]);
             *(u32x4*)(P + planes_at(pl, col, c, cols_pad, c_pad)) = o;
         }
     }
@@ -685,12 +723,16 @@
     return g;
 }
 
-template <int NP, int NS, int MINB, int ACT, bool KB2 = false, bool F16S = false>
+template <int NP, int NS, int MINB, int ACT, bool KB2 = false, bool F16S = false, int OF = 0>
 int launch_gemm_act(const AliveGemm& d, hipStream_t s) {
     constexpr int LDS = NS * 2 * NP * PLANE_BYTES;
+    auto* const kernel = [] {
+        if constexpr (OF == 0) return gemm_planes_kernel<NP, NS, MINB, ACT, KB2, F16S>;
+        else return gemm_planes_fmt_kernel<NP, NS, MINB, ACT, KB2, F16S, OF>;
+    }();
     {
         static LdsOptIn optin;
-        hipError_t e = optin.ensure({(const void*)gemm_planes_kernel<NP, NS, MINB, ACT, KB2, F16S>}, LDS);
+        hipError_t e = optin.ensure({(const void*)kernel}, LDS);
         if (e != hipSuccess) {
             alive_set_error("alive_gemm_planes: hipFuncSetAttribute: %s", hipGetErrorString(e));
             return ALIVE_ERR_LAUNCH;
@@ -699,7 +741,7 @@
     const int64_t cols = (int64_t)d.N * d.T;
     const int n_mt = cdiv(d.Co, GM), n_ct = cdiv(cols, GN);
     const int ntiles = n_mt * n_ct;
-    gemm_planes_kernel<NP, NS, MINB, ACT, KB2, F16S><<<ntiles, 256, LDS, s>>>(
+    kernel<<<ntiles, 256, LDS, s>>>(
         d, n_mt, ntiles, cols, pad_cols(cols), (d.Co + 15) & ~15, pad32(ACT == 4 ? d.Co / 2 : d.Co), pad32(d.Ci), make_walk(d),
         g_stamps);
     ALIVE_CHECK_LAUNCH("alive_gemm_planes");
@@ -785,6 +827,17 @@
     else if (planes == 2) to_planes_kernel<2><<<g, 256, 0, (hipStream_t)stream>>>(X, C, T, cols, cp, c_pad, (unsigned short*)P);
     else to_planes_kernel<3><<<g, 256, 0, (hipStream_t)stream>>>(X, C, T, cols, cp, c_pad, (unsigned short*)P);
     ALIVE_CHECK_LAUNCH("alive_to_planes");
+    return ALIVE_OK;
+}
+
+extern "C" int alive_sin_conv_planes(const float* W, int K_pad, const float* bias, const float* X, int N, int C, int T, void* P, void* stream) {
+    ALIVE_CHECK_ARG(W && X && P && N > 0 && C > 0 && T > 0 && K_pad >= 1, "alive_sin_conv_planes: bad args");
+    ALIVE_CHECK_ARG((((uintptr_t)P) & 15) == 0, "alive_sin_conv_planes: P must be 16-byte aligned");
+    const int64_t cols = (int64_t)N * T, cp = pad_cols(cols);
+    const int c_pad = pad32(C);
+    dim3 g((unsigned)(cp / 64), cdiv(c_pad, 64));
+    sin_planes_kernel<<<g, 256, 0, (hipStream_t)stream>>>(W, K_pad, bias, X, C, cols, cp, c_pad, (unsigned short*)P);
+    ALIVE_CHECK_LAUNCH("alive_sin_conv_planes");
     return ALIVE_OK;
 }
 
@@ -820,8 +873,19 @@
     const bool can_persist = ntiles >= 512 && variant != 1 &&
                              (d->b_row == 0 ? (int64_t)d->planes * pad_cols((int64_t)d->N * d->T) * pad32(d->Ci)
                                             : (int64_t)d->planes * d->b_plane) * 2 < (1ll << 32);
+    ALIVE_CHECK_ARG(d->pout_fmt >= 0 && d->pout_fmt <= 3, "alive_gemm_planes: pout_fmt %d (0: the operands' format, 1: one fp16 plane, 2 / 3: bf16 planes)",
+                    d->pout_fmt);
+    const int of = (d->pout_fmt == d->planes && !d->f16s) ? 0 : d->pout_fmt;
+    if (of != 0) {
+        const bool kb2 = d->planes == 1 && (pad32(d->Ci) & 63) == 0 && pad32(d->Ci) >= 128;
+        ALIVE_CHECK_ARG(d->Pout && d->act == 0 && d->b_row == 0 &&
+                        ((of == 1 && d->planes == 2 && !d->f16s) || (of == 2 && kb2) || (of == 3 && d->planes == 2 && d->f16s)),
+                        "alive_gemm_planes: pout_fmt %d from planes %d%s, act %d: built are act 0 with 2 bf16 planes -> 1, one fp16 plane "
+                        "(Ci a multiple of 64 from 128 on) -> 2, fp16 split planes -> 3", of, d->planes, d->f16s ? " (f16s)" : "", d->act);
+    }
     if (d->planes == 1) {
         if ((pad32(d->Ci) & 63) == 0 && pad32(d->Ci) >= 128) {
+            if (of == 2) return launch_gemm_act<2, 2, 2, 0, true, false, 2>(*d, (hipStream_t)stream);
             if (d->act == 1) return launch_gemm_act<2, 2, 2, 1, true>(*d, (hipStream_t)stream);
             if (d->act == 2) return launch_gemm_act<2, 2, 2, 2, true>(*d, (hipStream_t)stream);
             return launch_gemm_act<2, 2, 2, 0, true>(*d, (hipStream_t)stream);
@@ -829,15 +893,17 @@
         return launch_gemm<1, 4, 2>(*d, (hipStream_t)stream);
     }
     ALIVE_CHECK_ARG(!d->f16s || (d->planes == 2 && d->wscale != nullptr && d->in_unscale > 0.0f && d->act >= 0 && d->act <= 3 &&
-                                 (d->Pout == nullptr || d->pout_scale > 0.0f) && d->y_split == 0),
+                                 (d->Pout == nullptr || d->pout_scale > 0.0f || of != 0) && d->y_split == 0),
                     "alive_gemm_planes: f16s (fp16 split planes) takes planes = 2, wscale, in_unscale > 0, act 0 - 3 and pout_scale > 0 with Pout");
     if (d->planes == 2 && d->f16s) {
+        if (of == 3) return launch_gemm_act<2, 2, 2, 0, false, true, 3>(*d, (hipStream_t)stream);
         if (d->act == 3) return launch_gemm_act<2, 2, 2, 3, false, true>(*d, (hipStream_t)stream);
         if (d->act == 1) return launch_gemm_act<2, 2, 2, 1, false, true>(*d, (hipStream_t)stream);
         if (d->act == 2) return launch_gemm_act<2, 2, 2, 2, false, true>(*d, (hipStream_t)stream);
         return launch_gemm_act<2, 2, 2, 0, false, true>(*d, (hipStream_t)stream);
     }
     if (d->planes == 2) {
+        if (of == 1) return launch_gemm_act<2, 2, 2, 0, false, false, 1>(*d, (hipStream_t)stream);
         return launch_gemm<2, 2, 2>(*d, (hipStream_t)stream);
     }
     if (can_persist && nsteps >= 3) return launch_gemm_lw<3, 3>(*d, (hipStream_t)stream);
diff --git a/alive-vc_amd/csrc/networks.hip b/alive-vc_amd/csrc/networks.hip
--- a/alive-vc_amd/csrc/networks.hip
+++ b/alive-vc_amd/csrc/networks.hip
@@ -167,11 +167,11 @@
 inline size_t planes_bytes(int N, int T, int C, int planes) { return align_up(alive_planes_bytes((int64_t)N * T, C, planes), 256); }
 
 int pw_gemm(const float* W, const float* b, const void* P, int N, int T, int Ci, int Co, int planes, int act,
-            const float* post_add, const float* ch_scale, const float* residual, float* Y, void* Pout, void* s) {
+            const float* post_add, const float* ch_scale, const float* residual, float* Y, void* Pout, void* s, int pout_fmt = 0) {
     AliveGemm g;
     memset(&g, 0, sizeof(g));
     g.W = W; g.bias = b; g.P = P; g.N = N; g.T = T; g.Ci = Ci; g.Co = Co; g.planes = planes; g.act = act;
-    g.post_add = post_add; g.ch_scale = ch_scale; g.residual = residual; g.Y = Y; g.Pout = Pout;
+    g.post_add = post_add; g.ch_scale = ch_scale; g.residual = residual; g.Y = Y; g.Pout = Pout; g.pout_fmt = pout_fmt;
     return alive_gemm_planes(&g, s);
 }
 
@@ -186,7 +186,8 @@
 constexpr float F16S_ACT_SCALE = 256.0f;
 
 int convnext_layer(const ConvNeXtW& w, float* x, float* ybuf, float* hbuf, void* Pa, void* Ph, int N, int C, int H, int T,
-                   const float* cond, int cond_rows, int scale_row, int shift_row, int planes, void* s) {
+                   const float* cond, int cond_rows, int scale_row, int shift_row, int planes, void* s, void* Px = nullptr,
+                   int px_fmt = 0) {
     if (Pa != nullptr && planes == 3 && w.ws1 != nullptr && encoder_precision() == 1) {
         RUN(alive_dwconv_norm_planes_f16s(x, N, C, T, w.dw_w, w.dw_b, cond ? 1 : 0, w.gain, w.offset, cond, cond_rows, scale_row,
                                           shift_row, NORM_EPS, F16S_ACT_SCALE, Pa, s));
@@ -199,7 +200,7 @@
         memset(&g, 0, sizeof(g));
         g.W = (const float*)((const unsigned short*)w.pw2W + (size_t)3 * ((C + 15) & ~15) * ((H + 31) & ~31));
         g.bias = w.pw2b; g.P = Ph; g.N = N; g.T = T; g.Ci = H; g.Co = C; g.planes = 2; g.act = 0;
-        g.ch_scale = w.scale; g.residual = x; g.Y = x;
+        g.ch_scale = w.scale; g.residual = x; g.Y = Px != nullptr ? nullptr : x; g.Pout = Px; g.pout_fmt = Px != nullptr ? px_fmt : 0;
         g.f16s = 1; g.wscale = w.ws2; g.in_unscale = 1.0f / F16S_ACT_SCALE;
         return alive_gemm_planes(&g, s);
     }
@@ -210,7 +211,7 @@
         const float* W1 = gp == 1 ? plain_w(w.pw1W, (H + 15) & ~15, (C + 31) & ~31) : w.pw1W;
         const float* W2 = gp == 1 ? plain_w(w.pw2W, (C + 15) & ~15, (H + 31) & ~31) : w.pw2W;
         RUN(pw_gemm(W1, w.pw1b, Pa, N, T, C, H, gp, 1, nullptr, nullptr, nullptr, nullptr, Ph, s));
-        return pw_gemm(W2, w.pw2b, Ph, N, T, H, C, gp, 0, nullptr, w.scale, x, x, nullptr, s);
+        return pw_gemm(W2, w.pw2b, Ph, N, T, H, C, gp, 0, nullptr, w.scale, x, Px != nullptr ? nullptr : x, Px, s, Px != nullptr ? px_fmt : 0);
     }
     RUN(alive_dwconv_norm(x, N, C, T, w.dw_w, w.dw_b, cond ? 1 : 0, w.gain, w.offset, cond, cond_rows, scale_row,
                           shift_row, NORM_EPS, ybuf, s));
@@ -386,26 +387,34 @@
 }
 
 namespace {
-int ce_body(Table& t, EncBuffers& b, int N, int T, float* out, void* stream);
+int ce_body(Table& t, EncBuffers& b, int N, int T, float* out, void* stream, bool resident = true);
 int pe_body(Table& t, EncBuffers& b, int N, int T, float* f0, void* stream, float* logits = nullptr);
 }
 
 extern "C" size_t alive_content_encoder_workspace_bytes(int N, int T) { return enc_layout(nullptr, N, T, CE_C, CE_H, 0).bytes; }
-extern "C" int alive_content_encoder(const float* const* w, const float* spec, int N, int T, float* out, void* ws, void* stream) {
+static int content_encoder_run(const float* const* w, const float* spec, int N, int T, float* out, void* ws, void* stream, bool resident) {
     ALIVE_CHECK_ARG(w && spec && out && ws && N > 0 && T > 0, "alive_content_encoder: bad args");
     Table t(w);
     EncBuffers b = enc_layout(ws, N, T, CE_C, CE_H, 0);
     const float* inW = t.next(); const float* inb = t.next();
     RUN(pw_conv(inW, inb, spec, b.Pa, N, T, BINS, CE_C, 3, 0, nullptr, b.x, stream));
-    return ce_body(t, b, N, T, out, stream);
+    return ce_body(t, b, N, T, out, stream, resident);
+}
+extern "C" int alive_content_encoder(const float* const* w, const float* spec, int N, int T, float* out, void* ws, void* stream) {
+    return content_encoder_run(w, spec, N, T, out, ws, stream, true);
+}
+extern "C" int alive_content_encoder_ref(const float* const* w, const float* spec, int N, int T, float* out, void* ws, void* stream) {
+    return content_encoder_run(w, spec, N, T, out, ws, stream, false);
 }
 namespace {
-int ce_body(Table& t, EncBuffers& b, int N, int T, float* out, void* stream) {
+int ce_body(Table& t, EncBuffers& b, int N, int T, float* out, void* stream, bool resident) {
+    void* Px = resident ? b.Pa : nullptr;
     for (int i = 0; i < 4; ++i) {
         ConvNeXtW cw(t, false);
-        RUN(convnext_layer(cw, b.x, b.y, b.h, b.Pa, b.Ph, N, CE_C, CE_H, T, nullptr, 0, 0, 0, 3, stream));
+        RUN(convnext_layer(cw, b.x, b.y, b.h, b.Pa, b.Ph, N, CE_C, CE_H, T, nullptr, 0, 0, 0, 3, stream, i == 3 ? Px : nullptr, 3));
     }
     const float* oW = t.next(); const float* ob = t.next();
+    if (Px != nullptr) return pw_gemm(oW, ob, Px, N, T, CE_C, CE_OUT, 3, 0, nullptr, nullptr, nullptr, out, nullptr, stream);
     return pw_conv(oW, ob, b.x, b.Pa, N, T, CE_C, CE_OUT, 3, 0, nullptr, out, stream);
 }
 }
@@ -576,28 +585,40 @@
 }
 
 int decoder_run(const float* const* w, const float* x_in, const float* f0, const float* f0_win, const float* phi_in, int crop0,
-                int phi_col, int N, int Lf, int Lw_frames, int f_begin, float* wave, float* phi_out, DecBuffers& b, void* stream) {
+                int phi_col, int N, int Lf, int Lw_frames, int f_begin, float* wave, float* phi_out, DecBuffers& b, void* stream,
+                bool resident = true) {
     const bool ranged = Lf != Lw_frames;
     Table t(w);
     const int Lw = Lf * SEG;
+    resident = resident && b.Pa != nullptr;
     const float* inW = t.next(); const float* inb = t.next();
     RUN(pw_conv(inW, inb, x_in, b.Pa, N, Lf, 768, DEC_C, 2, 0, nullptr, b.x, stream));
     const float* c1W = t.next(); const float* c1b = t.next(); const float* c2W = t.next(); const float* c2b = t.next();
-    { AliveConv d = pw_desc(c1W, c1b, f0, N, 1, Lf, DEC_C, b.sinb); d.act = 3; RUN(alive_conv1d(&d, stream)); }
-    RUN(pw_conv(c2W, c2b, b.sinb, b.Pa, N, Lf, DEC_C, DEC_C, 2, 0, nullptr, b.cond, stream));
     const float* nfW = t.next(); const float* nfb = t.next();
-    if (b.Pa != nullptr && (decoder_bf16_mask() & 4)) {
-        RUN(alive_to_planes(b.cond, N, DEC_C, Lf, 1, b.Pa, stream));
-        RUN(pw_gemm(plain_w(nfW, 4096, DEC_C), nfb, b.Pa, N, Lf, DEC_C, 4096, 1, 0, nullptr, nullptr, nullptr, b.normfilm, nullptr, stream));
+    if (resident) {
+        const int cp = (decoder_bf16_mask() & 4) ? 1 : 2;
+        RUN(alive_sin_conv_planes(c1W, pad16(1), c1b, f0, N, DEC_C, Lf, b.Pa, stream));
+        RUN(pw_gemm(c2W, c2b, b.Pa, N, Lf, DEC_C, DEC_C, 2, 0, nullptr, nullptr, nullptr, nullptr, b.Ph, stream, cp));
+        RUN(pw_gemm(cp == 1 ? plain_w(nfW, 4096, DEC_C) : nfW, nfb, b.Ph, N, Lf, DEC_C, 4096, cp, 0, nullptr, nullptr, nullptr, b.normfilm,
+                    nullptr, stream));
     } else {
-        RUN(pw_conv(nfW, nfb, b.cond, b.Pa, N, Lf, DEC_C, 4096, 2, 0, nullptr, b.normfilm, stream));
+        { AliveConv d = pw_desc(c1W, c1b, f0, N, 1, Lf, DEC_C, b.sinb); d.act = 3; RUN(alive_conv1d(&d, stream)); }
+        RUN(pw_conv(c2W, c2b, b.sinb, b.Pa, N, Lf, DEC_C, DEC_C, 2, 0, nullptr, b.cond, stream));
+        if (b.Pa != nullptr && (decoder_bf16_mask() & 4)) {
+            RUN(alive_to_planes(b.cond, N, DEC_C, Lf, 1, b.Pa, stream));
+            RUN(pw_gemm(plain_w(nfW, 4096, DEC_C), nfb, b.Pa, N, Lf, DEC_C, 4096, 1, 0, nullptr, nullptr, nullptr, b.normfilm, nullptr, stream));
+        } else {
+            RUN(pw_conv(nfW, nfb, b.cond, b.Pa, N, Lf, DEC_C, 4096, 2, 0, nullptr, b.normfilm, stream));
+        }
     }
     for (int i = 0; i < 4; ++i) {
         ConvNeXtW cw(t, true);
-        RUN(convnext_layer(cw, b.x, b.y, b.h, b.Pa, b.Ph, N, DEC_C, DEC_H, Lf, b.normfilm, 4096, i * 1024, i * 1024 + 512, 2, stream));
+        RUN(convnext_layer(cw, b.x, b.y, b.h, b.Pa, b.Ph, N, DEC_C, DEC_H, Lf, b.normfilm, 4096, i * 1024, i * 1024 + 512, 2, stream,
+                           resident && i == 3 ? b.Pa : nullptr, 2));
     }
     const float* aW = t.next(); const float* ab = t.next();
-    RUN(pw_conv(aW, ab, b.x, b.Pa, N, Lf, DEC_C, NH, 2, 2, nullptr, b.amps, stream));
+    if (resident) RUN(pw_gemm(aW, ab, b.Pa, N, Lf, DEC_C, NH, 2, 2, nullptr, nullptr, nullptr, b.amps, nullptr, stream));
+    else RUN(pw_conv(aW, ab, b.x, b.Pa, N, Lf, DEC_C, NH, 2, 2, nullptr, b.amps, stream));
     RUN(alive_oscillator_range(b.amps, f0_win, phi_in, N, NH, Lw_frames, SEG, SR, crop0, phi_col, f_begin, Lf, b.src, phi_out, b.osc_ws, stream));
     const float* fW = t.next(); const float* fb = t.next(); const float* fpost = t.next();
     if (b.Pa != nullptr) {
@@ -819,6 +840,12 @@
     DecBuffers b = dec_layout(ws, N, Lf);
     return decoder_run(w, x_in, f0, f0, phi_in, crop0, phi_col, N, Lf, Lf, 0, wave, phi_out, b, stream);
 }
+extern "C" int alive_decoder_forward_ref(const float* const* w, const float* x_in, const float* f0, const float* phi_in, int crop0,
+                                         int phi_col, int N, int Lf, float* wave, float* phi_out, void* ws, void* stream) {
+    ALIVE_CHECK_ARG(w && x_in && f0 && wave && ws && N > 0 && Lf >= 5, "alive_decoder_forward_ref: bad args");
+    DecBuffers b = dec_layout(ws, N, Lf);
+    return decoder_run(w, x_in, f0, f0, phi_in, crop0, phi_col, N, Lf, Lf, 0, wave, phi_out, b, stream, false);
+}
 
 extern "C" int alive_decoder_forward_range(const float* const* w, const float* x_in, const float* f0, int N, int Lf, int f_begin,
                                            int n_frames, float* wave, void* ws, void* stream) {
diff --git a/alive-vc_amd/module/_native.py b/alive-vc_amd/module/_native.py
--- a/alive-vc_amd/module/_native.py
+++ b/alive-vc_amd/module/_native.py
@@ -34,6 +34,7 @@
         ("arg_val", C.c_void_p), ("arg_idx", C.c_void_p),
         ("Y2", C.c_void_p), ("y_split", C.c_int),
         ("f16s", C.c_int), ("wscale", C.c_void_p), ("in_unscale", C.c_float), ("pout_scale", C.c_float),
+        ("pout_fmt", C.c_int),
     ]
 
 
@@ -103,6 +104,7 @@
     "alive_planes_bytes": (_SZ, [_I64, _I, _I]),
     "alive_to_planes": (_I, [_VP, _I, _I, _I, _I, _VP, _VP]),
     "alive_gemm_planes": (_I, [C.POINTER(AliveGemm), _VP]),
+    "alive_sin_conv_planes": (_I, [_VP, _I, _VP, _VP, _I, _I, _I, _VP, _VP]),
     "alive_argmax_merge": (_I, [_VP, _VP, _I, _I64, _VP, _VP]),
     "alive_filter_block_small_weights": (_I, [_I]),
     "alive_filter_block_small": (_I, [_VP, _I, _I, _I, _VP, _VP, _I, _I, _I, _VP, _VP, _VP]),
@@ -147,6 +149,7 @@
     "alive_front_end": (_I, [_VP, _VP, _VP, _VP, _VP, _VP, _I, _I, _VP, _VP, _VP, _VP]),
     "alive_content_encoder_workspace_bytes": (_SZ, [_I, _I]),
     "alive_content_encoder": (_I, [_VP, _VP, _I, _I, _VP, _VP, _VP]),
+    "alive_content_encoder_ref": (_I, [_VP, _VP, _I, _I, _VP, _VP, _VP]),
     "alive_f0_estimate_workspace_bytes": (_SZ, [_I, _I]),
     "alive_f0_estimate": (_I, [_VP, _VP, _I, _I, _VP, _VP, _VP]),
     "alive_f0_logits": (_I, [_VP, _VP, _I, _I, _VP, _VP, _VP]),
@@ -154,6 +157,7 @@
     "alive_f0_track_rows": (_I, [_VP, _I, _I, _I, _I, _I, _VP, _VP, _VP, _VP, _VP, _VP, _VP, _VP, _VP, _VP]),
     "alive_decoder_workspace_bytes": (_SZ, [_I, _I]),
     "alive_decoder_forward": (_I, [_VP, _VP, _VP, _VP, _I, _I, _I, _I, _VP, _VP, _VP, _VP]),
+    "alive_decoder_forward_ref": (_I, [_VP, _VP, _VP, _VP, _I, _I, _I, _I, _VP, _VP, _VP, _VP]),
     "alive_decoder_forward_range": (_I, [_VP, _VP, _VP, _I, _I, _I, _I, _VP, _VP, _VP]),
     "alive_pitch_transform": (_I, [_VP, _I, _I, _I, _F, _F, _F, _VP]),
     "alive_pitch_transform_rows": (_I, [_VP, _I, _I, _I, _VP, _VP, _VP, _VP]),
diff --git a/include/alive_vc.h b/include/alive_vc.h
--- a/include/alive_vc.h
+++ b/include/alive_vc.h
@@ -196,8 +196,10 @@
     int f16s;
     const float* wscale;
     float in_unscale, pout_scale;
+    int pout_fmt;
 } AliveGemm;
 int alive_gemm_planes(const AliveGemm* desc, void* stream);
+int alive_sin_conv_planes(const float* W, int K_pad, const float* bias, const float* X, int N, int C, int T, void* P, void* stream);
 int alive_argmax_merge(const float* arg_val, const int32_t* arg_idx, int nblk, int64_t cols, float* out, void* stream);
 
 int alive_filter_block_small_weights(int C);
@@ -300,6 +302,8 @@
 size_t alive_content_encoder_workspace_bytes(int N, int T);
 int alive_content_encoder(const float* const* w, const float* spec, int N, int T,
                           float* out, void* ws, void* stream);
+int alive_content_encoder_ref(const float* const* w, const float* spec, int N, int T,
+                              float* out, void* ws, void* stream);
 
 size_t alive_f0_estimate_workspace_bytes(int N, int T);
 int alive_f0_estimate(const float* const* w, const float* spec, int N, int T,
@@ -322,6 +326,9 @@
 int alive_decoder_forward(const float* const* w, const float* x, const float* f0,
                           const float* phi_in, int crop0, int phi_col, int N, int Lf,
                           float* wave, float* phi_out, void* ws, void* stream);
+int alive_decoder_forward_ref(const float* const* w, const float* x, const float* f0,
+                              const float* phi_in, int crop0, int phi_col, int N, int Lf,
+                              float* wave, float* phi_out, void* ws, void* stream);
 
 int alive_pitch_transform(float* f0, int N, int T, int mode, float f0_rate, float pitch_shift,
                           float intonation, void* stream);
```

Result: no change. 1.329 million (median of 2 runs) (+0.2%).
